# tingliu/glia

Hardware: AMD Instinct MI355X
Metric: region_merges_per_sec (higher is better)
Workload: dtype u32 labels / f32 image / f64 statistics and features

## Files before the change

### glia_amd/csrc/greedy.hip

```cpp
#include <atomic>
#include <cstring>
#include <vector>
#include <limits>
#include <rocprim/device/device_scan.hpp>
#include <rocprim/device/device_radix_sort.hpp>
#include <rocprim/device/device_segmented_radix_sort.hpp>

#include "greedy_batch.hpp"

namespace glia {

__global__ void pq_build_level_kernel(PqTree t, int l) {
  const int lane = threadIdx.x & 63;
  uint32_t j = (blockIdx.x * blockDim.x + threadIdx.x) >> 6;
  if (j < t.lv[l].size) (void)pq_recompute_node(t, l, j, lane, true);
}

int pq_setup(DeviceBuffers& buf, PqTree& t, hipStream_t stream) {
  t.nlevels = 0;
  uint32_t n = t.nleaves;
  while (true) {
    n = (n + kFan - 1) / kFan;
    if (t.nlevels >= kMaxLevels) { set_error("greedy: edge table too large"); return GLIA_HMT_ERR_ARG; }
    PqLevel& L = t.lv[t.nlevels++];
    L.size = n;
    int rc;
    if ((rc = buf.get(&L.sal, n, false, stream))) return rc;
    if ((rc = buf.get(&L.seq, n, false, stream))) return rc;
    if ((rc = buf.get(&L.arg, n, false, stream))) return rc;
    if ((rc = buf.get(&L.dirty, n, true, stream))) return rc;
    if (n <= kTopMax) break;
  }
  {
    int rc;
    if ((rc = buf.get(&t.glist[0], t.lv[0].size, false, stream))) return rc;
    if ((rc = buf.get(&t.glist[1], t.lv[0].size, false, stream))) return rc;
    if ((rc = buf.get(&t.gcount, 2, true, stream))) return rc;
  }
  for (int l = 0; l < t.nlevels; ++l) {
    unsigned long long threads = (unsigned long long)t.lv[l].size * 64ull;
    hipLaunchKernelGGL(pq_build_level_kernel, dim3((unsigned)((threads + 255) / 256)), dim3(256), 0, stream, t, l);
  }
  GLIA_HIP_TRY(hipGetLastError());
  return GLIA_HMT_OK;
}

namespace {

__global__ void win_range_kernel(const double* sal, uint32_t E0, unsigned long long* mm) {
  unsigned long long lo = ~0ull, hi = 0ull;
  for (uint32_t i = blockIdx.x * blockDim.x + threadIdx.x; i < E0; i += gridDim.x * blockDim.x) {
    const unsigned long long b = f64_ord(sal[i]);
    lo = b < lo ? b : lo; hi = b > hi ? b : hi;
  }
  atomicMin(&mm[0], lo); atomicMax(&mm[1], hi);
}
__global__ void win_params_kernel(const unsigned long long* mm, uint32_t B, double* range) {
  const double smin = f64_unord(mm[0]), smax = f64_unord(mm[1]);
  range[0] = smin;
  range[1] = smax > smin ? (double)B / (smax - smin) : 0.0;
}
__global__ void win_collect_kernel(const EdgeRec* er, uint32_t n_edges, const uint8_t* rdead, unsigned long long* kseq, uint32_t* vals, uint32_t* counter) {
  const uint32_t e = blockIdx.x * blockDim.x + threadIdx.x;
  if (e >= n_edges) return;
  const unsigned long long q = er[e].seq;
  if (q == 0) return;
  const uint2 uv = *reinterpret_cast<const uint2*>(&er[e].u);
  if (rdead[uv.x] | rdead[uv.y]) return;
  const uint32_t i = atomicAdd(counter, 1u);
  kseq[i] = q; vals[i] = e;
}
__global__ void win_salkey_kernel(const EdgeRec* er, const uint32_t* vals, uint32_t n, unsigned long long* ksal) {
  const uint32_t i = blockIdx.x * blockDim.x + threadIdx.x;
  if (i < n) ksal[i] = f64_ord(er[vals[i]].sal);
}
__global__ void win_baseline_fill_kernel(WinState st, uint32_t n, uint32_t* isort_w, unsigned long long* isort_seq) {
  const uint32_t i = blockIdx.x * blockDim.x + threadIdx.x;
  if (i >= n) return;
  const EdgeRec r = st.er[isort_w[i]];
  isort_seq[i] = r.seq;
  atomicAdd(&st.wcnt[win_cell(r.sal, st.wrange[0], st.wrange[1], st.wB)], 1u);
}
__global__ void win_segments_kernel(WinState st, const uint32_t* isort, uint32_t n, uint32_t* ige) {
  const uint32_t c = blockIdx.x * blockDim.x + threadIdx.x;
  if (c > st.wB) return;
  uint32_t lo = 0, hi = n;
  while (lo < hi) {
    const uint32_t mid = (lo + hi) >> 1;
    if (win_cell(st.er[isort[mid]].sal, st.wrange[0], st.wrange[1], st.wB) >= c) lo = mid + 1; else hi = mid;
  }
  ige[c] = c == 0 ? n : lo;
}
__global__ void adj_fill_fat(GreedyState g, WinState st, uint32_t E0, uint32_t* cursor) {
  const uint32_t e = blockIdx.x * blockDim.x + threadIdx.x;
  if (e >= E0) return;
  const uint32_t u = g.e_u[e], v = g.e_v[e];
  const uint32_t pu = atomicAdd(&cursor[u], 1u), pv = atomicAdd(&cursor[v], 1u);
  const uint32_t ou = g.adj_off[u], ov = g.adj_off[v], lu = g.adj_len[u], lv = g.adj_len[v];
  FatEntry a; a.eid = e; a.rs = v; a.n = (uint32_t)g.e_n[e]; a.pos = pv; a.off = ov; a.len = lv; a.mean = g.e_mean[e];
  FatEntry b = a; b.rs = u; b.pos = pu; b.off = ou; b.len = lu;
  st.fpool[ou + pu] = a; g.e_posu[e] = pu;
  st.fpool[ov + pv] = b; g.e_posv[e] = pv;
  EdgeRec r; r.u = u; r.v = v; r.posu = pu; r.posv = pv; r.mean = g.e_mean[e]; r.n = g.e_n[e]; r.next = kNone;
  r.hu = make_uint2(ou, lu); r.hv = make_uint2(ov, lv); r.sal = g.pq.leaf_sal[e]; r.seq = g.pq.leaf_seq[e];
  st.er[e] = r;
}
__global__ void fat_to_thin(const FatEntry* f, uint2* out, unsigned long long n) {
  const unsigned long long i = (unsigned long long)blockIdx.x * blockDim.x + threadIdx.x;
  if (i < n) { const FatEntry fe = f[i]; out[i] = make_uint2(fe.eid, fe.eid == kNone ? 0u : fe.rs); }
}
__global__ void edge_unpack(GreedyState g, const EdgeRec* er, const uint8_t* rdead, uint32_t n) {
  const uint32_t e = blockIdx.x * blockDim.x + threadIdx.x;
  if (e >= n) return;
  const EdgeRec r = er[e];
  g.e_u[e] = r.u; g.e_v[e] = r.v; g.e_posu[e] = r.posu; g.e_posv[e] = r.posv; g.e_mean[e] = r.mean; g.e_n[e] = r.n;
  g.pq.leaf_sal[e] = r.sal; g.pq.leaf_seq[e] = (rdead[r.u] | rdead[r.v]) ? 0ull : r.seq;
}

__global__ void edge_flags(const uint32_t* pa, const uint32_t* pb, long long P, uint32_t* flag, long long* partner) {
  long long i = (long long)blockIdx.x * blockDim.x + threadIdx.x;
  if (i >= P) return;
  uint32_t a = pa[i], b = pb[i];
  long long j = (a < b) ? find_pair(pa, pb, P, b, a) : -1;
  flag[i] = j >= 0 ? 1u : 0u;
  partner[i] = j;
}

__global__ void edge_fill(const uint32_t* pa, const uint32_t* pb, const uint32_t* prec, long long P,
                          const uint32_t* flag, const uint32_t* eidx, const long long* partner,
                          const uint32_t* rlabel, uint32_t R, GreedyState st, uint32_t* deg) {
  long long i = (long long)blockIdx.x * blockDim.x + threadIdx.x;
  if (i >= P || !flag[i]) return;
  const uint32_t e = eidx[i];
  const long long j = partner[i];
  const uint32_t u = find_label(rlabel, R, pa[i]), v = find_label(rlabel, R, pb[i]);
  const uint32_t* wi = &prec[(size_t)i * kPairWords];
  const uint32_t* wj = &prec[(size_t)j * kPairWords];
  double si, sj;
  memcpy(&si, &wi[P_SUM], 8);
  memcpy(&sj, &wj[P_SUM], 8);
  const int n = (int)(wi[P_CNT] + wj[P_CNT]);
  const double mean = sdivide(si + sj, (double)n, 0.0);
  st.e_u[e] = u; st.e_v[e] = v; st.e_mean[e] = mean; st.e_n[e] = n;
  st.pq.leaf_sal[e] = -mean; st.pq.leaf_seq[e] = (unsigned long long)e + 1ull;
  atomicAdd(&deg[u], 1u);
  atomicAdd(&deg[v], 1u);
}

__global__ void adj_fill(GreedyState st, uint32_t E0, uint32_t* cursor) {
  uint32_t e = blockIdx.x * blockDim.x + threadIdx.x;
  if (e >= E0) return;
  const uint32_t u = st.e_u[e], v = st.e_v[e];
  const uint32_t pu = atomicAdd(&cursor[u], 1u), pv = atomicAdd(&cursor[v], 1u);
  st.pool[st.adj_off[u] + pu] = make_uint2(e, v); st.e_posu[e] = pu;
  st.pool[st.adj_off[v] + pv] = make_uint2(e, u); st.e_posv[e] = pv;
}

__global__ void region_sizes(const uint32_t* rrec, uint32_t R, unsigned long long* rsz, double* rsum) {
  uint32_t r = blockIdx.x * blockDim.x + threadIdx.x;
  if (r >= R) return;
  const uint32_t* w = &rrec[(size_t)r * kRegionWords];
  rsz[r] = w[R_CNT];
  double d; memcpy(&d, &w[R_SUM], 8); rsum[r] = d;
}

__global__ void median_collect(VolumeRef vol, const uint32_t* pa, const uint32_t* pb, long long P, const uint32_t* flag,
                               const uint32_t* eidx, const unsigned long long* e_off, uint32_t* cursor, float* out) {
  const long long N = vol.nx * vol.ny * vol.nz;
  const long long p = (long long)blockIdx.x * blockDim.x + threadIdx.x;
  if (p >= N) return;
  const long long x = p % vol.nx, y = (p / vol.nx) % vol.ny, z = p / (vol.nx * vol.ny);
  const uint32_t t = vol.lab[p];
  if (t == kMaskedLabel) return;
  uint32_t nb = t;
  const long long sy = vol.nx, sz = vol.nx * vol.ny;
  const uint32_t* L = vol.lab_nb;
  do {
    uint32_t q;
    if (x > 0 && (q = L[p - 1]) != t && q != kMaskedLabel) { nb = q; break; }
    if (x + 1 < vol.nx && (q = L[p + 1]) != t && q != kMaskedLabel) { nb = q; break; }
    if (y > 0 && (q = L[p - sy]) != t && q != kMaskedLabel) { nb = q; break; }
    if (y + 1 < vol.ny && (q = L[p + sy]) != t && q != kMaskedLabel) { nb = q; break; }
    if (vol.dim == 3) {
      if (z > 0 && (q = L[p - sz]) != t && q != kMaskedLabel) { nb = q; break; }
      if (z + 1 < vol.nz && (q = L[p + sz]) != t && q != kMaskedLabel) { nb = q; break; }
    }
  } while (false);
  if (nb == t) return;
  const long long i = find_pair(pa, pb, P, t < nb ? t : nb, t < nb ? nb : t);
  if (i < 0 || !flag[i]) return;
  const uint32_t e = eidx[i];
  out[e_off[e] + atomicAdd(&cursor[e], 1u)] = vol.pb[p];
}

__global__ void median_from_runs(const unsigned long long* pv_off, const float* pv, unsigned long long nV, const uint32_t* pa, const uint32_t* pb, long long P,
                                 const uint32_t* flag, const uint32_t* eidx, const unsigned long long* e_off, float* out) {
  const unsigned long long v = (unsigned long long)blockIdx.x * blockDim.x + threadIdx.x;
  if (v >= nV) return;
  long long lo = 0, hi = P;
  while (lo < hi) { const long long mid = (lo + hi) >> 1; if (pv_off[mid + 1] <= v) lo = mid + 1; else hi = mid; }
  const long long i = lo;
  const uint32_t a = pa[i], b = pb[i];
  const long long owner = a < b ? i : find_pair(pa, pb, P, b, a);
  if (owner < 0 || !flag[owner]) return;
  const unsigned long long first = owner == i ? 0ull : pv_off[owner + 1] - pv_off[owner];
  out[e_off[eidx[owner]] + first + (v - pv_off[i])] = pv[v];
}

__global__ void median_init(GreedyState st, uint32_t E0) {
  const uint32_t e = blockIdx.x * blockDim.x + threadIdx.x;
  if (e >= E0) return;
  const uint32_t n = (uint32_t)st.e_n[e];
  const double med = (double)st.vals[st.e_off[e] + n / 2u];
  st.e_mean[e] = med;
  st.pq.leaf_sal[e] = st.size_weight ? -med * (double)min(st.rsz[st.e_u[e]], st.rsz[st.e_v[e]]) : -med;
  atomicAdd(&st.rbv[st.e_u[e]], (unsigned long long)n);
  atomicAdd(&st.rbv[st.e_v[e]], (unsigned long long)n);
}

__global__ void fill_leaves_dead(PqTree t, uint32_t from) {
  uint32_t i = from + blockIdx.x * blockDim.x + threadIdx.x;
  if (i < t.nleaves) { t.leaf_seq[i] = 0; t.leaf_sal[i] = -__builtin_inf(); }
}

}

struct WinBaseline {
  unsigned long long *kseq = nullptr, *kseq2 = nullptr, *ksal = nullptr, *ksal2 = nullptr, *iseq = nullptr;
  uint32_t *vals = nullptr, *vals2 = nullptr, *isort = nullptr, *ige = nullptr, *counter = nullptr;
  void* tmp = nullptr; size_t tmp_bytes = 0;
  uint32_t E0 = 0;
  double h_range[2] = {0.0, 0.0};
  long long prev_top_cell = -1;
  unsigned long long prev_ne = 0;
  double horizon_factor = 0.0;

  int init(DeviceBuffers& buf, WinState& ws, const double* leaf_sal, uint32_t n_initial, uint32_t B, uint32_t R, hipStream_t stream) {
    int rc;
    E0 = n_initial;
    unsigned long long* mm; double* range;
    if ((rc = buf.get(&ws.rdead, 2 * (size_t)R, true, stream))) return rc;
    if ((rc = buf.get(&ws.whead, B, false, stream))) return rc;
    if ((rc = buf.get(&ws.wcnt, B, true, stream))) return rc;
    if ((rc = buf.get(&isort, E0, false, stream))) return rc;
    if ((rc = buf.get(&iseq, E0, false, stream))) return rc;
    if ((rc = buf.get(&ige, (size_t)B + 1, false, stream))) return rc;
    if ((rc = buf.get(&mm, 2, false, stream))) return rc;
    if ((rc = buf.get(&range, 2, false, stream))) return rc;
    if ((rc = buf.get(&kseq, E0, false, stream))) return rc;
    if ((rc = buf.get(&kseq2, E0, false, stream))) return rc;
    if ((rc = buf.get(&ksal, E0, false, stream))) return rc;
    if ((rc = buf.get(&ksal2, E0, false, stream))) return rc;
    if ((rc = buf.get(&vals, E0, false, stream))) return rc;
    if ((rc = buf.get(&vals2, E0, false, stream))) return rc;
    if ((rc = buf.get(&counter, 1, true, stream))) return rc;
    GLIA_HIP_TRY(rocprim::radix_sort_pairs_desc(nullptr, tmp_bytes, kseq, kseq2, vals, vals2, (size_t)E0, 0, 64, stream));
    if ((rc = buf.get((char**)&tmp, tmp_bytes ? tmp_bytes : 16, false, stream))) return rc;
    ws.wrange = range; ws.isort = isort; ws.isort_seq = iseq; ws.ige = ige;
    const unsigned long long mm0[2] = {~0ull, 0ull};
    GLIA_HIP_TRY(hipMemcpyAsync(mm, mm0, sizeof(mm0), hipMemcpyHostToDevice, stream));
    hipLaunchKernelGGL(win_range_kernel, dim3(256), dim3(256), 0, stream, leaf_sal, E0, mm);
    hipLaunchKernelGGL(win_params_kernel, dim3(1), dim3(1), 0, stream, mm, B, range);
    GLIA_HIP_TRY(hipGetLastError());
    GLIA_HIP_TRY(hipMemcpyAsync(h_range, range, sizeof(h_range), hipMemcpyDeviceToHost, stream));
    GLIA_HIP_TRY(hipStreamSynchronize(stream));
    return GLIA_HMT_OK;
  }
  int rebaseline(WinState& ws, uint32_t n_edges, unsigned long long* ctrl, hipStream_t stream) {
    GLIA_HIP_TRY(hipMemsetAsync(counter, 0, sizeof(uint32_t), stream));
    hipLaunchKernelGGL(win_collect_kernel, dim3((n_edges + 255) / 256), dim3(256), 0, stream, ws.er, n_edges, ws.rdead, kseq, vals, counter);
    uint32_t n = 0;
    GLIA_HIP_TRY(hipMemcpyAsync(&n, counter, sizeof(uint32_t), hipMemcpyDeviceToHost, stream));
    GLIA_HIP_TRY(hipStreamSynchronize(stream));
    if (n > E0) { set_error("greedy: more live edges than initial edges (internal error)"); return GLIA_HMT_ERR_INTERNAL; }
    if (n) {
      size_t bytes = tmp_bytes;
      GLIA_HIP_TRY(rocprim::radix_sort_pairs_desc(tmp, bytes, kseq, kseq2, vals, vals2, (size_t)n, 0, 64, stream));
      hipLaunchKernelGGL(win_salkey_kernel, dim3((n + 255) / 256), dim3(256), 0, stream, ws.er, vals2, n, ksal);
      bytes = tmp_bytes;
      GLIA_HIP_TRY(rocprim::radix_sort_pairs_desc(tmp, bytes, ksal, ksal2, vals2, isort, (size_t)n, 0, 64, stream));
    }
    GLIA_HIP_TRY(hipMemsetAsync(ws.whead, 0xFF, sizeof(uint32_t) * ws.wB, stream));
    GLIA_HIP_TRY(hipMemsetAsync(ws.wcnt, 0, sizeof(uint32_t) * ws.wB, stream));
    if (n) hipLaunchKernelGGL(win_baseline_fill_kernel, dim3((n + 255) / 256), dim3(256), 0, stream, ws, n, isort, iseq);
    hipLaunchKernelGGL(win_segments_kernel, dim3((ws.wB + 1 + 255) / 256), dim3(256), 0, stream, ws, isort, n, ige);
    GLIA_HIP_TRY(hipGetLastError());
    ws.nsort = n;
    std::string renv;
    ws.rebase_after = option("GLIA_HMT_REBASE", &renv) ? strtoull(renv.c_str(), nullptr, 10) : std::max<unsigned long long>(800000ull, (unsigned long long)n / 2ull);
    ws.wch = 0;
    if (horizon_factor > 0.0 && n > 4096) {
      unsigned long long topkey = 0;
      GLIA_HIP_TRY(hipMemcpyAsync(&topkey, ksal2, sizeof(topkey), hipMemcpyDeviceToHost, stream));
      GLIA_HIP_TRY(hipStreamSynchronize(stream));
      const long long top_cell = (long long)win_cell(f64_unord(topkey), h_range[0], h_range[1], ws.wB);
      if (prev_top_cell >= 0 && n_edges > prev_ne) {
        const double d = (double)std::max<long long>(0, prev_top_cell - top_cell);
        const double delta = std::max(horizon_factor * d * (double)ws.rebase_after / (double)(n_edges - prev_ne), (double)ws.wB / 512.0);
        ws.wch = (double)top_cell > delta ? (uint32_t)((double)top_cell - delta) : 0u;
      }
      prev_top_cell = top_cell; prev_ne = n_edges;
    }
    ws.ne_base = n_edges;
    const double inf = std::numeric_limits<double>::infinity();
    ctrl[CTRL_CTHR] = (unsigned long long)(long long)(ws.wB - 1);
    memcpy(&ctrl[CTRL_TSAL], &inf, 8); ctrl[CTRL_TSEQ] = ~0ull; ctrl[CTRL_IPTR] = 0;
    return GLIA_HMT_OK;
  }
};

static int run_pb_loop(const RagArrays& rag, hipStream_t stream, const PbRequest& req, MergeResult* out) {
  const long long P = rag.P;
  const uint32_t R = (uint32_t)rag.R;
  if (R == 0 || P == 0) return GLIA_HMT_OK;
  const VolumeRef* median_of = req.median_of;
  CallEvents<3> ev;
  int rc;
  if ((rc = ev.create())) return rc;
  GLIA_HIP_TRY(hipEventRecord(ev.ev[0], stream));
  DeviceBuffers buf;
  uint32_t* flag; uint32_t* eidx; long long* partner;
  if ((rc = buf.get(&flag, P + 1, true, stream))) return rc;
  if ((rc = buf.get(&eidx, P + 1, false, stream))) return rc;
  if ((rc = buf.get(&partner, P, false, stream))) return rc;
  hipLaunchKernelGGL(edge_flags, dim3((unsigned)((P + 255) / 256)), dim3(256), 0, stream, rag.d_pa, rag.d_pb, P, flag, partner);
  if ((rc = rocprim_run(buf, stream, [&](void* t, size_t& b) {
        return rocprim::exclusive_scan(t, b, flag, eidx, 0u, (size_t)(P + 1), rocprim::plus<uint32_t>(), stream); }))) return rc;
  uint32_t E0 = 0;
  GLIA_HIP_TRY(hipMemcpyAsync(&E0, eidx + P, sizeof(uint32_t), hipMemcpyDeviceToHost, stream));
  GLIA_HIP_TRY(hipStreamSynchronize(stream));
  if (E0 == 0) return GLIA_HMT_OK;

  GreedyState st;
  memset(&st, 0, sizeof(st));
  st.R0 = R;
  const bool mincap = initial_capacities(E0, 18, 36, &st.Ecap, &st.pool_cap);
  if ((rc = buf.get(&st.adj_off, 2 * (size_t)R, true, stream))) return rc;
  if ((rc = buf.get(&st.adj_len, 2 * (size_t)R + 1, true, stream))) return rc;
  std::string o_window, o_batch, o_txt;
  const bool batch_off = option("GLIA_HMT_PB_BATCH", &o_batch) && o_batch[0] == '0';
  bool window = !median_of && !req.size_weight && !(option("GLIA_HMT_PB_WINDOW", &o_window) && o_window[0] == '0');
  WinState ws;
  memset(&ws, 0, sizeof(ws));
  GrowList edges, entries, values;
  if (window) {
    if ((rc = entries.add(buf, &ws.fpool, st.pool_cap, stream))) return rc;
    if ((rc = edges.add(buf, &ws.er, st.Ecap, stream))) return rc;
  }
  else if ((rc = entries.add(buf, &st.pool, st.pool_cap, stream))) return rc;
  if ((rc = edges.add(buf, &st.e_u, st.Ecap, stream)) || (rc = edges.add(buf, &st.e_v, st.Ecap, stream)) ||
      (rc = edges.add(buf, &st.e_posu, st.Ecap, stream)) || (rc = edges.add(buf, &st.e_posv, st.Ecap, stream)) ||
      (rc = edges.add(buf, &st.e_mean, st.Ecap, stream)) || (rc = edges.add(buf, &st.e_n, st.Ecap, stream, true)) ||
      (rc = edges.add(buf, &st.pq.leaf_sal, st.Ecap, stream)) || (rc = edges.add(buf, &st.pq.leaf_seq, st.Ecap, stream)))
    return rc;
  st.pq.nleaves = st.Ecap;
  if ((rc = buf.get(&st.rsz, 2 * (size_t)R, true, stream))) return rc;
  if ((rc = buf.get(&st.rsum, 2 * (size_t)R, true, stream))) return rc;
  st.cond_n = req.cond_n; st.cond_rpb = req.cond_rpb; st.size_weight = req.size_weight ? 1 : 0;
  st.cond_t0 = req.cond_n > 0 ? (unsigned long long)req.cond_sizes[0] : 0; st.cond_t1 = req.cond_n > 1 ? (unsigned long long)req.cond_sizes[1] : 0;
  hipLaunchKernelGGL(region_sizes, dim3((R + 255) / 256), dim3(256), 0, stream, rag.d_rrec, R, st.rsz, st.rsum);
  if ((rc = buf.get(&st.mark0, 2 * (size_t)R, true, stream))) return rc;
  if ((rc = buf.get(&st.mark1, 2 * (size_t)R, true, stream))) return rc;
  if ((rc = buf.get(&st.order, 3 * ((size_t)R + 16), false, stream))) return rc;
  if ((rc = buf.get(&st.sal_out, (size_t)R + 16, false, stream))) return rc;
  if ((rc = buf.get(&st.ctrl, 16, true, stream))) return rc;
  uint32_t* cursor;
  if ((rc = buf.get(&cursor, 2 * (size_t)R, true, stream))) return rc;

  hipLaunchKernelGGL(fill_leaves_dead, dim3((st.Ecap - E0 + 255) / 256), dim3(256), 0, stream, st.pq, E0);
  hipLaunchKernelGGL(edge_fill, dim3((unsigned)((P + 255) / 256)), dim3(256), 0, stream, rag.d_pa, rag.d_pb, rag.d_prec, P,
                     flag, eidx, partner, rag.d_rlabel, R, st, st.adj_len);
  if ((rc = rocprim_run(buf, stream, [&](void* t, size_t& b) {
        return rocprim::exclusive_scan(t, b, st.adj_len, st.adj_off, 0u, (size_t)R, rocprim::plus<uint32_t>(), stream); }))) return rc;
  if (window) hipLaunchKernelGGL(adj_fill_fat, dim3((E0 + 255) / 256), dim3(256), 0, stream, st, ws, E0, cursor);
  else hipLaunchKernelGGL(adj_fill, dim3((E0 + 255) / 256), dim3(256), 0, stream, st, E0, cursor);
  GLIA_HIP_TRY(hipGetLastError());
  unsigned long long n_values = 0;
  if (median_of) {
    if ((rc = edges.add(buf, &st.e_off, st.Ecap, stream))) return rc;
    if ((rc = buf.get(&st.rbv, 2 * (size_t)R, true, stream))) return rc;
    if ((rc = rocprim_run(buf, stream, [&](void* t, size_t& b) {
          return rocprim::exclusive_scan(t, b, st.e_n, st.e_off, 0ull, (size_t)E0 + 1, rocprim::plus<unsigned long long>(), stream); }))) return rc;
    GLIA_HIP_TRY(hipMemcpyAsync(&n_values, st.e_off + E0, sizeof(n_values), hipMemcpyDeviceToHost, stream));
    GLIA_HIP_TRY(hipStreamSynchronize(stream));
    if (n_values >= 0xFFFFFFFFull) { set_error("merge_order_pb: more than 2^32 boundary voxels (median linkage)"); return GLIA_HMT_ERR_ARG; }
    st.vals_cap = mincap ? std::max(n_values, 1ull) : n_values * 4ull + (1ull << 20);
    float* unsorted;
    if ((rc = values.add(buf, &st.vals, (size_t)st.vals_cap, stream))) return rc;
    if ((rc = buf.get(&unsorted, (size_t)n_values, false, stream))) return rc;
    uint32_t* vcursor;
    if ((rc = buf.get(&vcursor, (size_t)E0, true, stream))) return rc;
    if (median_of->lab) {
      const long long N = median_of->nx * median_of->ny * median_of->nz;
      hipLaunchKernelGGL(median_collect, dim3((unsigned)((N + 255) / 256)), dim3(256), 0, stream, *median_of, rag.d_pa, rag.d_pb, P,
                         flag, eidx, st.e_off, vcursor, unsorted);
    } else {
      if (!rag.d_pv_off) { set_error("merge_order_pb: median linkage needs the volume or the map's boundary values"); return GLIA_HMT_ERR_UNSUPPORTED; }
      if (rag.nV) hipLaunchKernelGGL(median_from_runs, dim3((unsigned)((rag.nV + 255) / 256)), dim3(256), 0, stream, rag.d_pv_off, rag.d_pv, rag.nV, rag.d_pa, rag.d_pb,
                                     (long long)P, flag, eidx, st.e_off, unsorted);
    }
    GLIA_HIP_TRY(hipGetLastError());
    if ((rc = rocprim_run(buf, stream, [&](void* t, size_t& b) {
          return rocprim::segmented_radix_sort_keys(t, b, unsorted, st.vals, (unsigned)n_values, (unsigned)E0, st.e_off, st.e_off + 1, 0, 32, stream); }))) return rc;
    hipLaunchKernelGGL(median_init, dim3((E0 + 255) / 256), dim3(256), 0, stream, st, E0);
    GLIA_HIP_TRY(hipGetLastError());
  }
  unsigned long long ctrl[CTRL_WORDS] = {};
  ctrl[CTRL_EDGES] = E0; ctrl[CTRL_ENTRIES] = 2ull * E0; ctrl[CTRL_STATUS] = ST_RUN; ctrl[CTRL_VALUES] = n_values;
  WinBaseline base;
  if (window) {
    uint32_t B = 256;
    while (B < E0 / 4 && B < (1u << 22)) B <<= 1;
    ws.wB = B; ws.R0 = R;
    ws.wcap = kWinCap; ws.wbudget = kWinBudget;
    ws.force_tree = 0;
    if (option("GLIA_HMT_FORCE_TREE", &o_txt)) ws.force_tree = strtoull(o_txt.c_str(), nullptr, 10);
    if (option("GLIA_HMT_WINCAP", &o_txt)) {
      const uint32_t c = (uint32_t)strtoul(o_txt.c_str(), nullptr, 10);
      if (c >= 16 && c <= kWinCap) { ws.wcap = c; ws.wbudget = c / 2; }
    }
    ws.order = st.order; ws.sal_out = st.sal_out; ws.ctrl = st.ctrl; ws.rsz = st.rsz; ws.rsum = st.rsum;
    ws.mark0 = st.mark0; ws.mark1 = st.mark1; ws.adj_off = st.adj_off; ws.adj_len = st.adj_len;
    ws.pool_cap = st.pool_cap; ws.Ecap = st.Ecap;
    ws.cond_n = st.cond_n; ws.cond_t0 = st.cond_t0; ws.cond_t1 = st.cond_t1; ws.cond_rpb = st.cond_rpb;
    if ((rc = base.init(buf, ws, st.pq.leaf_sal, E0, B, R, stream))) return rc;
    if (req.cond_n <= 0 && !batch_off) base.horizon_factor = option("GLIA_HMT_HORIZON", &o_txt) ? atof(o_txt.c_str()) : 0.5;
    if ((rc = base.rebaseline(ws, E0, ctrl, stream))) return rc;
  } else if ((rc = pq_setup(buf, st.pq, stream))) return rc;
  GLIA_HIP_TRY(hipMemcpyAsync(st.ctrl, ctrl, sizeof(ctrl), hipMemcpyHostToDevice, stream));
  GLIA_HIP_TRY(hipEventRecord(ev.ev[1], stream));


  st.max_iters = window ? 1ull << 22 : 1ull << 16;
  const bool trace = option("GLIA_HMT_TRACE");
  if (option("GLIA_HMT_MAXITERS", &o_txt)) st.max_iters = std::max(1ull, strtoull(o_txt.c_str(), nullptr, 10));
  const auto kernel = [&]() { return !window ? "tree" : req.cond_n > 0 ? "window" : "batch"; };
  const auto unhandled = [&]() {
    set_error(std::string("greedy: the ") + kernel() + " kernel stopped with status " + std::to_string(ctrl[CTRL_STATUS]) + ", which its driver does not handle (internal error)");
    return GLIA_HMT_ERR_INTERNAL;
  };
  while (true) {
    if (window) {
      ws.max_iters = st.max_iters;
      if (req.cond_n > 0) hipLaunchKernelGGL(greedy_window_kernel<true>, dim3(1), dim3(kGreedyThreads), 0, stream, ws);
      else if (batch_off) hipLaunchKernelGGL(greedy_window_kernel<false>, dim3(1), dim3(kGreedyThreads), 0, stream, ws);
      else hipLaunchKernelGGL(greedy_batch_kernel, dim3(1), dim3(kGreedyThreads), 0, stream, ws);
    } else if (median_of) hipLaunchKernelGGL(greedy_pb_kernel<true>, dim3(1), dim3(kGreedyThreads), 0, stream, st);
    else hipLaunchKernelGGL(greedy_pb_kernel<false>, dim3(1), dim3(kGreedyThreads), 0, stream, st);
    GLIA_HIP_TRY(hipGetLastError());
    GLIA_HIP_TRY(hipMemcpyAsync(ctrl, st.ctrl, sizeof(ctrl), hipMemcpyDeviceToHost, stream));
    GLIA_HIP_TRY(hipStreamSynchronize(stream));
    if (trace) fprintf(stderr, "[trace] merge loop launch ended: status %llu, merges %llu of %u regions, edges %llu, list entries %llu\n", ctrl[CTRL_STATUS], ctrl[CTRL_MERGES], R, ctrl[CTRL_EDGES], ctrl[CTRL_ENTRIES]);
    if (ctrl[CTRL_STATUS] == ST_DONE) break;
    switch (ctrl[CTRL_STATUS]) {
      case ST_RUN:
        if (!window) continue;
        break;
      case ST_REBASE:
        if (!window) return unhandled();
        break;
      case ST_BAD_SALIENCY: set_error("Error: invalid boundary saliency..."); return GLIA_HMT_ERR_SALIENCY;
      case ST_INTERNAL: {
        char msg[256];
        snprintf(msg, sizeof(msg), "greedy: window queue overflow or more merges than regions (internal error: merges %llu of %u regions, %llu edges of %u initial, "
                 "window %llu%s, %s kernel)", ctrl[CTRL_MERGES], R, ctrl[CTRL_EDGES], E0, ctrl[CTRL_WFILL], ctrl[CTRL_WERR] ? " overflowed" : "", kernel());
        set_error(msg);
        return GLIA_HMT_ERR_INTERNAL;
      }
      case ST_NEED_TREE:
        if (!window) return unhandled();
        entries.remove(&ws.fpool);
        edges.remove(&ws.er);
        if ((rc = entries.add(buf, &st.pool, st.pool_cap, stream))) return rc;
        hipLaunchKernelGGL(fat_to_thin, dim3((unsigned)((ctrl[CTRL_ENTRIES] + 255) / 256)), dim3(256), 0, stream, ws.fpool, st.pool, ctrl[CTRL_ENTRIES]);
        hipLaunchKernelGGL(edge_unpack, dim3((unsigned)((ctrl[CTRL_EDGES] + 255) / 256)), dim3(256), 0, stream, st, ws.er, ws.rdead, (uint32_t)ctrl[CTRL_EDGES]);
        GLIA_HIP_TRY(hipGetLastError());
        if ((rc = pq_setup(buf, st.pq, stream))) return rc;
        window = false;
        st.max_iters = 1ull << 16;
        break;
      case ST_NEED_POOL: {
        const unsigned long long ncap = st.pool_cap * 2;
        if ((rc = entries.grow(buf, (size_t)st.pool_cap, (size_t)ncap, stream))) return rc;
        st.pool_cap = ncap; ws.pool_cap = ncap;
        break;
      }
      case ST_NEED_VALUES: {
        if (!median_of) return unhandled();
        const unsigned long long ncap = st.vals_cap * 2;
        if ((rc = values.grow(buf, (size_t)ctrl[CTRL_VALUES], (size_t)ncap, stream))) return rc;
        st.vals_cap = ncap;
        break;
      }
      case ST_NEED_EDGES: {
        if (st.Ecap >= kMaxEdgeSlots) { set_error("greedy: more than 2^32 edge slots needed"); return GLIA_HMT_ERR_ARG; }
        const uint32_t ocap = st.Ecap, ncap = (uint32_t)std::min<unsigned long long>(kMaxEdgeSlots, (unsigned long long)ocap * 2ull);
        if ((rc = edges.grow(buf, ocap, ncap, stream))) return rc;
        st.Ecap = ncap; st.pq.nleaves = ncap; ws.Ecap = ncap;
        hipLaunchKernelGGL(fill_leaves_dead, dim3((ncap - ocap + 255) / 256), dim3(256), 0, stream, st.pq, ocap);
        if (!window && (rc = pq_setup(buf, st.pq, stream))) return rc;
        break;
      }
      default: return unhandled();
    }
    if (window) {
      if ((rc = base.rebaseline(ws, (uint32_t)ctrl[CTRL_EDGES], ctrl, stream))) return rc;
      GLIA_HIP_TRY(hipMemcpyAsync(st.ctrl + CTRL_CTHR, ctrl + CTRL_CTHR, 4 * sizeof(unsigned long long), hipMemcpyHostToDevice, stream));
    }
    unsigned long long zero = ST_RUN;
    GLIA_HIP_TRY(hipMemcpyAsync(st.ctrl + CTRL_STATUS, &zero, sizeof(zero), hipMemcpyHostToDevice, stream));
  }
  GLIA_HIP_TRY(hipEventRecord(ev.ev[2], stream));
  GLIA_HIP_TRY(hipEventSynchronize(ev.ev[2]));
  out->ms_table = ev.ms(0, 1); out->ms_loop = ev.ms(1, 2);
  out->n_scored = (int64_t)ctrl[CTRL_EDGES];
  return copy_merges(out, (int64_t)ctrl[CTRL_MERGES], st.order, st.sal_out);
}


static std::atomic<unsigned long long> g_internal_errors{0};
unsigned long long internal_errors() { return g_internal_errors.load(); }
void count_internal_error() { g_internal_errors.fetch_add(1); }
bool merge_order_is_consistent(const uint32_t* o, int64_t n, uint32_t R, int64_t* first_bad) {
  std::vector<uint8_t> gone(2 * (size_t)R + 1, 0);
  for (int64_t k = 0; k < n; ++k) {
    const uint32_t a = o[3 * k], b = o[3 * k + 1], c = o[3 * k + 2];
    if (k >= (int64_t)R || c != R + (uint32_t)k || a >= c || b >= c || a == b || gone[a] || gone[b]) { if (first_bad) *first_bad = k; return false; }
    gone[a] = gone[b] = 1;
  }
  return true;
}
int finish_merge_order(int rc, const uint32_t* o, int64_t n, uint32_t R, hipStream_t stream) {
  int64_t bad = -1;
  if (rc == GLIA_HMT_OK && !merge_order_is_consistent(o, n, R, &bad)) {
    set_error("greedy: merge " + std::to_string(bad) + " of " + std::to_string(n) + " joins a region that does not exist (any more) or creates the wrong one (internal error)");
    rc = GLIA_HMT_ERR_INTERNAL;
  }
  if (rc == GLIA_HMT_ERR_INTERNAL) { count_internal_error(); (void)hipStreamSynchronize(stream); }
  return rc;
}
int greedy_mean(const RagArrays& rag, hipStream_t stream, const PbRequest& req, MergeResult* out) {
  const int rc = run_pb_loop(rag, stream, req, out);
  return finish_merge_order(rc, out->order.data(), out->n, (uint32_t)rag.R, stream);
}

}
```

### glia_amd/csrc/greedy_batch.hpp

```cpp
#pragma once
#include "greedy_window.hpp"

namespace glia {
namespace {

constexpr uint32_t kBatchKill = 32;
constexpr int kMemP = 3;
constexpr uint32_t kMemMax = 192;
struct BatchShared {
  alignas(16) Key part1[kNW];
  alignas(16) Key part2[kNW];
  uint32_t nkill, kovf; alignas(16) uint32_t kill[kBatchKill];
  uint32_t byrank[kNW];
  uint32_t bitmap[kNW][64];
  uint32_t m_newcount[kNW], m_total[kNW], m_ok[kNW];
  double m_maxsal[kNW];
  uint32_t bad;
};

template <int CTRL, int ROW_MASK = 0xf>
__device__ __forceinline__ void top2_ord_step(unsigned long long& a1, unsigned long long& a2) {
  const unsigned long long b1 = dpp64<CTRL, ROW_MASK, ROW_MASK != 0xf>(a1), b2 = dpp64<CTRL, ROW_MASK, ROW_MASK != 0xf>(a2);
  const bool g = b1 > a1;
  const unsigned long long hi = g ? b1 : a1, lo = g ? a1 : b1, m2 = b2 > a2 ? b2 : a2;
  a1 = hi; a2 = lo > m2 ? lo : m2;
}
__device__ __forceinline__ void wave_top2_ord(unsigned long long& a1, unsigned long long& a2) {
  top2_ord_step<0xB1>(a1, a2);
  top2_ord_step<0x4E>(a1, a2);
  top2_ord_step<0x124>(a1, a2);
  top2_ord_step<0x128>(a1, a2);
  top2_ord_step<0x142, 0xa>(a1, a2);
  top2_ord_step<0x143, 0xc>(a1, a2);
  a1 = lane_u64(a1, 63); a2 = lane_u64(a2, 63);
}

#ifdef GLIA_HMT_PROFILE
__device__ unsigned long long g_scanprof[8];
__device__ unsigned long long g_scanfill[3][3];
#define SCAN_T(i) do { if (tid == 0) { const unsigned long long tn_ = __builtin_readcyclecounter(); g_scanprof[i] += tn_ - st_; st_ = tn_; } } while (0)
#else
#define SCAN_T(i) do {} while (0)
#endif
enum { kScanOther = 0, kScanNarrow = 1, kScanWide = 2 };
__device__ __forceinline__ void batch_scan(const WinState& st, WinShared& w, BatchShared& b, int tid, [[maybe_unused]] int from) {
#ifdef GLIA_HMT_PROFILE
  unsigned long long st_ = __builtin_readcyclecounter();
  if (tid == 0) g_scanprof[7] += 1;
#endif
  const uint32_t n = w.n < st.wcap ? w.n : st.wcap, nk = b.nkill < kBatchKill ? b.nkill : kBatchKill, kovf = b.kovf;
#ifdef GLIA_HMT_PROFILE
  if (tid == 0) g_scanfill[from][n <= 512u ? 0 : n <= 1024u ? 1 : 2] += 1;
#endif
  const uint32_t own = 64u * (uint32_t)(((tid >> 6) + (tid & 63)) & 7) + (uint32_t)(tid & 63);
  Key k1, k2;
  k1.sal = -__builtin_inf(); k1.seq = 0; k1.arg = 0; k2 = k1;
  auto pass = [&](auto nb_tag) {
    constexpr int NB = decltype(nb_tag)::value;
    unsigned long long q[NB]; uint32_t e[NB]; double sl[NB];
#pragma unroll
    for (int j = 0; j < NB; ++j) { const uint32_t i = own + (uint32_t)j * kGreedyThreads; q[j] = w.seq[i]; e[j] = w.e[i]; sl[j] = w.sal[i]; }
    const uint4 ka = *reinterpret_cast<const uint4*>(&b.kill[0]), kb = *reinterpret_cast<const uint4*>(&b.kill[4]);
    const uint32_t kl[8] = {ka.x, ka.y, ka.z, ka.w, kb.x, kb.y, kb.z, kb.w};
    SCAN_T(0);
    uint32_t deadm[NB];
#pragma unroll
    for (int j = 0; j < NB; ++j) {
      uint32_t d = 0;
#pragma unroll
      for (uint32_t t = 0; t < 8; ++t) d |= (uint32_t)(t < nk) & (uint32_t)(kl[t] == e[j]);
      deadm[j] = d;
    }
    if (nk > 8u) {
      for (uint32_t t = 8; t < nk; ++t) {
        const uint32_t kt = b.kill[t];
#pragma unroll
        for (int j = 0; j < NB; ++j) deadm[j] |= (uint32_t)(kt == e[j]);
      }
      if (kovf) {
        full_barrier();
#pragma unroll
        for (int j = 0; j < NB; ++j) {
          const uint32_t i = own + (uint32_t)j * kGreedyThreads;
          if (i < n && q[j] != 0) deadm[j] |= (uint32_t)(st.er[e[j]].seq == 0);
        }
      }
    }
#pragma unroll
    for (int j = 0; j < NB; ++j) {
      const uint32_t i = own + (uint32_t)j * kGreedyThreads;
      const bool was = (i < n) & (q[j] != 0);
      const bool live = was & (deadm[j] == 0u);
      if (was & !live) w.seq[i] = 0;
      Key c; c.sal = live ? sl[j] : -__builtin_inf(); c.seq = live ? q[j] : 0ull; c.arg = i;
      const bool b1 = better(c, k1), b2 = better(c, k2);
      k2.sal = b1 ? k1.sal : (b2 ? c.sal : k2.sal); k2.seq = b1 ? k1.seq : (b2 ? c.seq : k2.seq); k2.arg = b1 ? k1.arg : (b2 ? c.arg : k2.arg);
      k1.sal = b1 ? c.sal : k1.sal; k1.seq = b1 ? c.seq : k1.seq; k1.arg = b1 ? c.arg : k1.arg;
    }
  };
  static_assert(kWinPer == 3, "batch_scan: one pass instance per number of blocks");
  const uint32_t nu = (uint32_t)__builtin_amdgcn_readfirstlane((int)n);
  if (nu > 2u * kGreedyThreads) pass(std::integral_constant<int, 3>{});
  else if (nu > kGreedyThreads) pass(std::integral_constant<int, 2>{});
  else pass(std::integral_constant<int, 1>{});
  SCAN_T(1);
  const int lane = tid & 63;
  const unsigned long long o1 = f64_ord(k1.sal), o2 = f64_ord(k2.sal);
  unsigned long long M1 = o1, M2 = o2;
  wave_top2_ord(M1, M2);
  const unsigned long long t1 = __ballot(o1 == M1), t1l = __ballot((o1 == M1) & (k1.seq != 0ull));
  const int l1 = (int)__builtin_ctzll(t1);
  const bool win1 = lane == l1;
  Key kk; kk.sal = win1 ? k2.sal : k1.sal; kk.seq = win1 ? k2.seq : k1.seq; kk.arg = win1 ? k2.arg : k1.arg;
  const unsigned long long oc = win1 ? o2 : o1;
  const unsigned long long t2 = __ballot(oc == M2), t2l = __ballot((oc == M2) & (kk.seq != 0ull));
  Key m1, m2;
  if (__popcll(t1) == 1 || t1l == 0ull) {
    m1 = lane_key(k1, l1);
    int src = (int)__builtin_ctzll(t2);
    if (__popcll(t2) != 1 && t2l != 0ull) {
#ifdef GLIA_HMT_PROFILE
      if (tid == 0) g_scanprof[5] += 1;
#endif
      const unsigned long long ms = wave_max_u64(oc == M2 ? kk.seq : 0ull);
      src = (int)__builtin_ctzll(__ballot((oc == M2) & (kk.seq == ms)));
    }
    m2 = lane_key(kk, src);
    SCAN_T(2);
  } else {
#ifdef GLIA_HMT_PROFILE
    if (tid == 0) g_scanprof[6] += 1;
#endif
    unsigned long long S1 = o1 == M1 ? k1.seq : 0ull, S2 = o2 == M1 ? k2.seq : 0ull;
    wave_top2_ord(S1, S2);
    const int w1 = (int)__builtin_ctzll(__ballot((o1 == M1) & (k1.seq == S1)));
    const bool winr = lane == w1;
    Key kc; kc.sal = winr ? k2.sal : k1.sal; kc.seq = winr ? k2.seq : k1.seq; kc.arg = winr ? k2.arg : k1.arg;
    const unsigned long long occ = winr ? o2 : o1;
    m1 = lane_key(k1, w1);
    m2 = lane_key(kc, (int)__builtin_ctzll(__ballot((occ == M1) & (kc.seq == S2))));
    SCAN_T(3);
  }
  if ((tid & 63) == 0) { b.part1[tid >> 6] = m1; b.part2[tid >> 6] = m2; }
  full_barrier();
  SCAN_T(4);
  if (tid == 0) { b.nkill = 0; b.kovf = 0; }
}

#ifdef GLIA_HMT_PROFILE
__device__ unsigned long long g_wideprof[8];
#define WIDE_T(i) do { if (tid == 0) { const unsigned long long tn_ = __builtin_readcyclecounter(); g_wideprof[i] += tn_ - wt_; wt_ = tn_; } } while (0)
#else
#define WIDE_T(i) do {} while (0)
#endif
__device__ __forceinline__ uint32_t batch_contract_wide(const WinState& st, WinShared& w, WinWork& s, BatchShared& b, int tid, uint32_t slot, double rootsal,
                                                      unsigned long long k, unsigned long long ne, unsigned long long pool_used, double smin, double scale, uint32_t* newcount_out) {
  const uint32_t e = w.e[slot], r0 = w.u[slot], r1 = w.v[slot];
  const uint2 h0r = w.hu[slot], h1r = w.hv[slot];
  const uint32_t wn_now = w.n;
  const uint32_t off0 = h0r.x, len0 = h0r.y, off1 = h1r.x, len1 = h1r.y;
  const uint32_t total = len0 + len1;
  const uint32_t r2 = st.R0 + (uint32_t)k;
  const uint32_t r2off = (uint32_t)pool_used;
#ifdef GLIA_HMT_PROFILE
  unsigned long long wt_ = __builtin_readcyclecounter();
#endif
  lds_barrier();
  WIDE_T(0);
  if (tid == 0) {
    w.seq[slot] = 0;
    st.order[3 * k + 0] = r0; st.order[3 * k + 1] = r1; st.order[3 * k + 2] = r2;
    st.sal_out[k] = rootsal;
    st.er[e].seq = 0;
    st.rdead[r0] = 1; st.rdead[r1] = 1;
  }
  const bool small = total <= kMarkMax;
  win_stage_lists(st, s, tid, e, off0, len0, off1, len1, small);
  if (small) lds_barrier(); else full_barrier();
  WIDE_T(1);
  if (wn_now + total > st.wcap && wn_now > st.wcap / 2u) win_compact(w, tid, st.wcap);
  WIDE_T(2);
  const WinTau tau = {w.cthr, w.tsal, w.tseq, smin, scale};
  const uint32_t nwork = small ? s.nitems : total;
  const uint32_t lenR2 = small ? nwork : 0u;
  bool bad = false;
  uint32_t pend_e = kNone, pend_old = kNone;
  auto rounds = [&](auto small_tag) {
    constexpr bool SMALL = decltype(small_tag)::value;
    for (uint32_t base = 0; base < nwork; base += kGreedyThreads) {
      const uint32_t i = base + tid;
      if (i >= nwork) break;
      FatEntry f0, f1;
      bool h0, h1;
      uint32_t rs;
      if (!win_match<SMALL>(st, s, i, e, off0, len0, off1, &rs, &h0, &h1, &f0, &f1)) continue;
      const uint32_t idx = atomicAdd(&s.newcount, 1u);
      const uint32_t newE = (uint32_t)ne + idx;
      double first;
      int second;
      if (mean_link(h0, f0.mean, (int)f0.n, h1, f1.mean, (int)f1.n, &first, &second)) bad = true;
      const uint32_t offRs = f0.off, posRs = f0.pos, lenRs = f0.len;
      if (h0 && h1) st.fpool[offRs + f1.pos].eid = kNone;
      const unsigned long long seq = update_seq(k, rs, r0, h0);
      const double sal = -first;
      store_new_edge(st, newE, rs, r2, posRs, idx, first, second, sal, seq, offRs, lenRs, r2off, lenR2);
      win_queue_edge<true>(st, w, tau, newE, sal, seq, rs, r2, make_uint2(offRs, lenRs), make_uint2(r2off, lenR2), pend_e, pend_old);
      if (h0) win_retire_edge<true, false, kBatchKill>(st, tau, f0.eid, -f0.mean, &b.nkill, b.kill, &b.kovf);
      if (h1) win_retire_edge<true, false, kBatchKill>(st, tau, f1.eid, -f1.mean, &b.nkill, b.kill, &b.kovf);
    }
  };
  if (small) rounds(std::true_type{}); else rounds(std::false_type{});
  if (bad) b.bad = 1;
  WIDE_T(3);
  if (small) lds_barrier(); else full_barrier();
  WIDE_T(4);
  const uint32_t newcount = s.newcount;
  if (!small) win_complete_r2(st, tid, (uint32_t)ne, r2off, newcount);
  if (!small) for (uint32_t i = tid; i < (w.n < st.wcap ? w.n : st.wcap); i += kGreedyThreads) if (w.v[i] == r2) w.hv[i].y = newcount;
  if (pend_e != kNone) st.er[pend_e].next = pend_old;
  if (tid == 0) { st.adj_off[r2] = r2off; st.adj_len[r2] = newcount; }
  lds_barrier();
  WIDE_T(5);
  if (tid == 0) { s.nitems = 0; s.newcount = 0; }
  *newcount_out = newcount;
  return total;
}

__global__ __launch_bounds__(kGreedyThreads) void greedy_batch_kernel(WinState st) {
  __shared__ WinShared w;
  __shared__ WinWork s;
  __shared__ BatchShared b;
  const int tid = threadIdx.x, lane = tid & 63, wave = tid >> 6;
  unsigned long long k = st.ctrl[CTRL_MERGES], ne = st.ctrl[CTRL_EDGES], pool_used = st.ctrl[CTRL_ENTRIES];
  uint32_t status = ST_RUN;
  win_enter(st, w, s, tid);
  if (tid == 0) { b.nkill = 0; b.kovf = 0; b.bad = 0; }
  b.bitmap[wave][lane] = 0;
  if (tid < kNW) { Key z; z.sal = -__builtin_inf(); z.seq = 0; z.arg = 0; b.part1[tid] = z; b.part2[tid] = z; }
  full_barrier();
  const double smin = st.wrange[0], scale = st.wrange[1];
  uint32_t pend_e = kNone, pend_old = kNone;
  constexpr uint32_t kTab = kMarkSlots / kNW;
  uint32_t* const tk = &s.mk[wave * kTab]; uint32_t* const t0 = &s.mv0[wave * kTab]; uint32_t* const t1 = &s.mv1[wave * kTab];
  static_assert(sizeof(s.stage) >= (size_t)kNW * kTab * 20, "per-wave staging");
  uint32_t* const sg_eid = reinterpret_cast<uint32_t*>(&s.stage[0]) + wave * kTab;
  uint32_t* const sg_n = reinterpret_cast<uint32_t*>(&s.stage[0]) + (kNW + wave) * kTab;
  uint32_t* const sg_pos = reinterpret_cast<uint32_t*>(&s.stage[0]) + (2 * kNW + wave) * kTab;
  double* const sg_mean = reinterpret_cast<double*>(reinterpret_cast<uint32_t*>(&s.stage[0]) + 3 * kNW * kTab) + wave * kTab;
#ifdef GLIA_HMT_PROFILE
  unsigned long long bph[8] = {0, 0, 0, 0, 0, 0, 0, 0}, blast = __builtin_readcyclecounter(), brounds = 0, bmembers = 0, bvalid = 0, bwide = 0, bcut_sal = 0, bcut_dep = 0;
  unsigned long long bw_n[4] = {0, 0, 0, 0}, bw_cyc[4] = {0, 0, 0, 0}, bw_ent[4] = {0, 0, 0, 0}, bw_new[4] = {0, 0, 0, 0};
  unsigned long long bsel[2] = {0, 0}, bsel_n[2] = {0, 0};
#define BPH0(wide) do { if (tid == 0) { unsigned long long tn = __builtin_readcyclecounter(); bph[0] += tn - blast; bsel[wide] += tn - blast; bsel_n[wide] += 1; blast = tn; } } while (0)
#define BPH(i) do { if (tid == 0) { unsigned long long tn = __builtin_readcyclecounter(); bph[i] += tn - blast; blast = tn; } } while (0)
#else
#define BPH(i) do {} while (0)
#define BPH0(wide) do {} while (0)
#endif

  for (unsigned long long it = 0; it < st.max_iters; ++it) {
    if (ne - st.ne_base > st.rebase_after) { status = ST_REBASE; break; }
    const int gi = lane >> 3, gj = lane & 7;
    const Key A = b.part1[gi], B = b.part1[gj], C = b.part2[gi];
    const unsigned long long beats = __ballot(better(A, B)), under = __ballot(better(C, B));
    const unsigned long long col = 0x0101010101010101ull << gj;
    const uint32_t rank = (uint32_t)__popcll(beats & col);
    const bool cand_ok = B.seq != 0 && (under & col) == 0;
    if (gi == 0 && cand_ok) b.byrank[rank] = (uint32_t)gj;
    const unsigned long long okmask = __ballot(gi == 0 && cand_ok);
    const uint32_t M = (uint32_t)__popcll(okmask);
    if (M == 0) {
      BPH(5);
      if (pend_e != kNone) { st.er[pend_e].next = pend_old; pend_e = kNone; }
      if (st.force_tree && k >= st.force_tree) { status = ST_NEED_TREE; break; }
      const int r = win_reload(st, w, tid, reinterpret_cast<double*>(&s.stage[0]), reinterpret_cast<unsigned long long*>(&s.stage[0]) + kSelMax);
      BPH(6);
      if (r == 1) { status = ST_DONE; break; }
      if (r == 2) { status = ST_NEED_TREE; break; }
      if (r == 3) { status = ST_REBASE; break; }
      batch_scan(st, w, b, tid, kScanOther);
      continue;
    }
    const unsigned long long minemask = __ballot(gi == 0 && cand_ok && rank == (uint32_t)wave);
    const bool member = minemask != 0;
    const int cj = member ? (int)__builtin_ctzll(minemask) : 0;
    const Key me = b.part1[cj];
    const uint32_t slot = me.arg;
    const uint32_t e = w.e[slot], r0 = w.u[slot], r1 = w.v[slot];
    const uint2 h0r = w.hu[slot], h1r = w.hv[slot];
    const uint32_t off0 = h0r.x, len0 = h0r.y, off1 = h1r.x, len1 = h1r.y;
    const uint32_t total = len0 + len1;
    if (k >= (unsigned long long)st.R0) { status = ST_INTERNAL; break; }
    const unsigned long long firstmask = __ballot(gi == 0 && cand_ok && rank == 0u);
    const Key top = b.part1[__builtin_ctzll(firstmask)];
    const uint2 th0 = w.hu[top.arg], th1 = w.hv[top.arg];
    const uint32_t top_total = th0.y + th1.y;
    BPH0(top_total > kMemMax ? 1 : 0);
    if (top_total > kMemMax) {
      if (ne + top_total > st.Ecap) { status = ST_NEED_EDGES; break; }
      if (pool_used + top_total > st.pool_cap) { status = ST_NEED_POOL; break; }
      uint32_t newcount = 0;
#ifdef GLIA_HMT_PROFILE
      const unsigned long long tw0 = __builtin_readcyclecounter();
#endif
      const uint32_t tt = batch_contract_wide(st, w, s, b, tid, top.arg, top.sal, k, ne, pool_used, smin, scale, &newcount);
      if (b.bad) { status = ST_BAD_SALIENCY; break; }
      k += 1; ne += newcount; pool_used += tt;
#ifdef GLIA_HMT_PROFILE
      bwide += 1;
      { const int cls = tt <= 512u ? 0 : tt <= kMarkMax ? 1 : tt <= 8192u ? 2 : 3; bw_n[cls] += 1; bw_cyc[cls] += __builtin_readcyclecounter() - tw0; bw_ent[cls] += tt; bw_new[cls] += newcount; }
#endif
      batch_scan(st, w, b, tid, kScanWide);
      if (w.spill_ord) { if (pend_e != kNone) { st.er[pend_e].next = pend_old; pend_e = kNone; } win_evict(st, w, tid); batch_scan(st, w, b, tid, kScanOther); }
      BPH(4);
      continue;
    }
    const bool narrow = member && total <= kMemMax;
    b.bitmap[wave][lane] = 0;
    FatEntry fe[kMemP];
    bool act[kMemP], side1[kMemP];
    uint32_t h[kMemP];
#pragma unroll
    for (int p = 0; p < kMemP; ++p) {
      const uint32_t i = (uint32_t)lane + 64u * (uint32_t)p;
      const bool inlist = narrow && i < total;
      side1[p] = i >= len0;
      fe[p].eid = kNone; fe[p].rs = 0; fe[p].n = 0; fe[p].pos = 0; fe[p].off = 0; fe[p].len = 0; fe[p].mean = 0.0;
      if (inlist) fe[p] = st.fpool[side1[p] ? off1 + (i - len0) : off0 + i];
      act[p] = inlist;
    }
    if (pend_e != kNone) { st.er[pend_e].next = pend_old; pend_e = kNone; }
#pragma unroll
    for (int p = 0; p < kMemP; ++p) {
      act[p] = act[p] && fe[p].eid != e && fe[p].eid != kNone;
      h[p] = (fe[p].rs * 2654435761u) >> 24;
      if (act[p]) {
        while (true) {
          const uint32_t old = atomicCAS(&tk[h[p]], 0u, fe[p].rs + 1u);
          if (old == 0u || old == fe[p].rs + 1u) break;
          h[p] = (h[p] + 1u) & (kTab - 1u);
        }
        if (side1[p]) {
          t1[h[p]] = 1u;
          sg_eid[h[p]] = fe[p].eid; sg_n[h[p]] = fe[p].n; sg_pos[h[p]] = fe[p].pos; sg_mean[h[p]] = fe[p].mean;
        } else t0[h[p]] = 1u;
        atomicOr(&b.bitmap[wave][(fe[p].rs >> 5) & 63u], 1u << (fe[p].rs & 31u));
      }
    }
    if (narrow && lane == 0) { atomicOr(&b.bitmap[wave][(r0 >> 5) & 63u], 1u << (r0 & 31u)); atomicOr(&b.bitmap[wave][(r1 >> 5) & 63u], 1u << (r1 & 31u)); }
    asm volatile("s_waitcnt lgkmcnt(0)" ::: "memory");
    bool owner[kMemP], both[kMemP];
    uint32_t p_eid[kMemP], p_n[kMemP], p_pos[kMemP];
    double p_mean[kMemP];
#pragma unroll
    for (int p = 0; p < kMemP; ++p) {
      const uint32_t m0 = act[p] ? t0[h[p]] : 0u, m1 = act[p] ? t1[h[p]] : 0u;
      owner[p] = act[p] && (!side1[p] || m0 == 0u);
      both[p] = owner[p] && !side1[p] && m1 != 0u;
      p_eid[p] = sg_eid[h[p]]; p_n[p] = sg_n[h[p]]; p_pos[p] = sg_pos[h[p]]; p_mean[p] = sg_mean[h[p]];
    }
#pragma unroll
    for (int p = 0; p < kMemP; ++p) if (act[p]) { tk[h[p]] = 0u; t0[h[p]] = 0u; t1[h[p]] = 0u; }
    double first[kMemP]; int second[kMemP]; uint32_t idx[kMemP];
    bool bad = false;
    uint32_t newcount = 0;
    double mx = -__builtin_inf();
#pragma unroll
    for (int p = 0; p < kMemP; ++p) {
      const bool h0 = owner[p] && !side1[p], h1 = owner[p] && (side1[p] || both[p]);
      bad = mean_link(h0, fe[p].mean, (int)fe[p].n, h1, both[p] ? p_mean[p] : fe[p].mean, both[p] ? (int)p_n[p] : (int)fe[p].n, &first[p], &second[p]) || bad;
      const double f = first[p];
      const unsigned long long ownmask = __ballot(owner[p]);
      idx[p] = newcount + (uint32_t)__popcll(ownmask & ((1ull << lane) - 1ull));
      newcount += (uint32_t)__popcll(ownmask);
      mx = (owner[p] && -f > mx) ? -f : mx;
    }
#pragma unroll
    for (int d = 32; d >= 1; d >>= 1) { const double o = __shfl_xor(mx, d); mx = o > mx ? o : mx; }
    if (lane == 0) { b.m_newcount[wave] = narrow ? newcount : 0u; b.m_total[wave] = narrow ? total : 0xFFFFFFFFu; b.m_maxsal[wave] = mx; }
    if (bad) b.bad = 1;
    const uint32_t wn_round = w.n;
    lds_barrier();
    BPH(1);
    if (b.bad) { status = ST_BAD_SALIENCY; break; }
    uint32_t V, ne_off, pool_off, my_ne, my_pool;
    {
      const uint32_t j = (uint32_t)lane & 7u;
      const Key kj = b.part1[b.byrank[j]];
      const uint32_t u = w.u[kj.arg], v = w.v[kj.arg];
      const uint32_t tj = b.m_total[j], nj = b.m_newcount[j];
      double pm = -__builtin_inf();
      uint32_t hit = 0, pre_n = 0, pre_t = 0;
#pragma unroll
      for (uint32_t i = 0; i < (uint32_t)kNW; ++i) {
        const double ms = b.m_maxsal[i];
        const uint32_t bu = b.bitmap[i][(u >> 5) & 63u], bv = b.bitmap[i][(v >> 5) & 63u];
        const uint32_t ti = b.m_total[i], ni = b.m_newcount[i];
        if (i < j) { pm = ms > pm ? ms : pm; hit |= ((bu >> (u & 31u)) | (bv >> (v & 31u))) & 1u; pre_n += ni; pre_t += ti; }
      }
      const bool okj = j < M && tj != 0xFFFFFFFFu && (j == 0u || (kj.sal > pm && hit == 0u));
      const uint32_t okbits = (uint32_t)(__ballot(lane < kNW && okj) & 0xFFull);
      V = (uint32_t)__builtin_ctz(~okbits);
#ifdef GLIA_HMT_PROFILE
      if (V < M) { const uint32_t cutsal = (uint32_t)(__ballot(lane < kNW && j == V && !(kj.sal > pm)) & 0xFFull); if (cutsal) bcut_sal += 1; else bcut_dep += 1; }
#endif
      my_ne = (uint32_t)__builtin_amdgcn_readlane((int)pre_n, wave); my_pool = (uint32_t)__builtin_amdgcn_readlane((int)pre_t, wave);
      const uint32_t last = V - 1u;
      ne_off = (uint32_t)__shfl((int)(pre_n + nj), (int)last); pool_off = (uint32_t)__shfl((int)(pre_t + tj), (int)last);
    }
    const uint32_t sum_tot = pool_off;
    if (ne + sum_tot > st.Ecap) { status = ST_NEED_EDGES; break; }
    if (pool_used + sum_tot > st.pool_cap) { status = ST_NEED_POOL; break; }
    bool popped = false;
    if (wn_round + ne_off > st.wcap && wn_round > st.wcap / 2u) {
      if ((uint32_t)wave < V && lane == 0) w.seq[slot] = 0;
      popped = true;
      lds_barrier();
      win_compact(w, tid, st.wcap);
    }
    const WinTau tau = {w.cthr, w.tsal, w.tseq, smin, scale};
    BPH(2);
    if ((uint32_t)wave < V) {
      const unsigned long long kk = k + (unsigned long long)wave;
      const uint32_t r2 = st.R0 + (uint32_t)kk;
      const uint32_t r2off = (uint32_t)pool_used + my_pool;
      if (lane == 0) {
        if (!popped) w.seq[slot] = 0;
        st.order[3 * kk + 0] = r0; st.order[3 * kk + 1] = r1; st.order[3 * kk + 2] = r2;
        st.sal_out[kk] = me.sal;
        st.er[e].seq = 0;
        st.rdead[r0] = 1; st.rdead[r1] = 1;
        st.adj_off[r2] = r2off; st.adj_len[r2] = newcount;
      }
#pragma unroll
      for (int p = 0; p < kMemP; ++p) {
        if (!owner[p]) continue;
        const bool h0 = !side1[p];
        const uint32_t rs = fe[p].rs;
        const uint32_t newE = (uint32_t)ne + my_ne + idx[p];
        const uint32_t offRs = fe[p].off, posRs = fe[p].pos, lenRs = fe[p].len;
        if (both[p]) st.fpool[offRs + p_pos[p]].eid = kNone;
        const unsigned long long seq = update_seq(kk, rs, r0, h0);
        const double sal = -first[p];
        store_new_edge(st, newE, rs, r2, posRs, idx[p], first[p], second[p], sal, seq, offRs, lenRs, r2off, newcount);
        win_queue_edge<true>(st, w, tau, newE, sal, seq, rs, r2, make_uint2(offRs, lenRs), make_uint2(r2off, newcount), pend_e, pend_old);
        win_retire_edge<true, false, kBatchKill>(st, tau, fe[p].eid, -fe[p].mean, &b.nkill, b.kill, &b.kovf);
        if (both[p]) win_retire_edge<true, false, kBatchKill>(st, tau, p_eid[p], -p_mean[p], &b.nkill, b.kill, &b.kovf);
      }
    }
    lds_barrier();
    BPH(3);
#ifdef GLIA_HMT_PROFILE
    brounds += 1; bmembers += M; bvalid += V;
#endif
    k += V; ne += ne_off; pool_used += pool_off;
    batch_scan(st, w, b, tid, kScanNarrow);
    if (w.spill_ord) { if (pend_e != kNone) { st.er[pend_e].next = pend_old; pend_e = kNone; } win_evict(st, w, tid); batch_scan(st, w, b, tid, kScanOther); }
    BPH(4);
  }
#ifdef GLIA_HMT_PROFILE
  if (tid == 0) printf("[batch profile] merges %llu: select %llu  compute %llu  validate %llu  commit %llu  scan %llu  loop-top %llu  reload %llu (cycles); rounds %llu candidates %llu committed %llu (cut by saliency %llu, by adjacency %llu) wide %llu\n",
                       k, bph[0], bph[1], bph[2], bph[3], bph[4], bph[5], bph[6], brounds, bmembers, bvalid, bcut_sal, bcut_dep, bwide);
  if (tid == 0) printf("[batch profile] scan phases (cumulative cycles, wave 0): loads %llu  compare %llu  top2 %llu  top2 with a tied best %llu  barrier %llu  calls %llu  tied second %llu  tied best %llu\n",
                       g_scanprof[0], g_scanprof[1], g_scanprof[2], g_scanprof[3], g_scanprof[4], g_scanprof[7], g_scanprof[5], g_scanprof[6]);
  if (tid == 0) printf("[batch profile] scan fill (cumulative; n <= 512, <= 1024, more): after reload/evict %llu %llu %llu  after narrow round %llu %llu %llu  after wide %llu %llu %llu\n",
                       g_scanfill[0][0], g_scanfill[0][1], g_scanfill[0][2], g_scanfill[1][0], g_scanfill[1][1], g_scanfill[1][2], g_scanfill[2][0], g_scanfill[2][1], g_scanfill[2][2]);
  if (tid == 0) printf("[batch profile] loop top (this launch): narrow rounds %llu cycles %llu  wide pops %llu cycles %llu\n", bsel_n[0], bsel[0], bsel_n[1], bsel[1]);
  if (tid == 0) printf("[batch profile] wide phases (cumulative cycles): entry-barrier %llu  lists+table %llu  compact %llu  main loop (wave 0) %llu  loop barrier %llu  tail %llu\n",
                       g_wideprof[0], g_wideprof[1], g_wideprof[2], g_wideprof[3], g_wideprof[4], g_wideprof[5]);
  if (tid == 0) printf("[batch profile] wide by entries (<=512, <=1408, <=8192, more): n %llu %llu %llu %llu  cycles %llu %llu %llu %llu  entries %llu %llu %llu %llu  new edges %llu %llu %llu %llu\n",
                       bw_n[0], bw_n[1], bw_n[2], bw_n[3], bw_cyc[0], bw_cyc[1], bw_cyc[2], bw_cyc[3], bw_ent[0], bw_ent[1], bw_ent[2], bw_ent[3], bw_new[0], bw_new[1], bw_new[2], bw_new[3]);
#endif
  if (pend_e != kNone) st.er[pend_e].next = pend_old;
  full_barrier();
  win_leave(st, w, tid, k, ne, pool_used, status);
}

}
}
```

### glia_amd/csrc/greedy_window.hpp

```cpp
#pragma once
#include "greedy_tree.hpp"

namespace glia {

struct __attribute__((aligned(16))) FatEntry {
  uint32_t eid;
  uint32_t rs;
  uint32_t n;
  uint32_t pos;
  uint32_t off;
  uint32_t len;
  double mean;
};

namespace {

struct __attribute__((aligned(16))) EdgeRec {
  uint32_t u, v, posu, posv;
  double mean; int n; uint32_t next;
  uint2 hu, hv;
  double sal; unsigned long long seq;
};
static_assert(sizeof(EdgeRec) == 64, "EdgeRec layout");
struct WinState {
  EdgeRec* er; FatEntry* fpool;
  uint32_t* whead;
  uint32_t* wcnt;
  const uint32_t* isort; const unsigned long long* isort_seq;
  const uint32_t* ige;
  const double* wrange;
  uint32_t* order; double* sal_out; unsigned long long* ctrl;
  unsigned long long* rsz; double* rsum; uint32_t *mark0, *mark1, *adj_off, *adj_len;
  unsigned long long pool_cap, max_iters, cond_t0, cond_t1;
  double cond_rpb;
  uint32_t R0, Ecap, wB, nsort;
  unsigned long long ne_base, rebase_after;
  uint32_t wcap, wbudget;
  int cond_n;
  uint32_t wch;
  uint8_t* rdead;
  unsigned long long force_tree;
};
constexpr uint32_t kWinCap = 1536;
constexpr uint32_t kWinBudget = 768;
constexpr uint32_t kWinMinLoad = 192;
constexpr uint32_t kWinMinPartial = 96;
constexpr uint32_t kKillMax = 8;
constexpr int kNW = kGreedyThreads / 64;
constexpr int kWinPer = (int)(kWinCap / kGreedyThreads);
static_assert(kWinPer * kGreedyThreads == (int)kWinCap, "window capacity");
struct WinShared {
  double sal[kWinCap];
  unsigned long long seq[kWinCap];
  uint32_t e[kWinCap], u[kWinCap], v[kWinCap];
  uint2 hu[kWinCap], hv[kWinCap];
  int cthr; uint32_t iptr;
  double tsal; unsigned long long tseq;
  alignas(16) uint32_t n;
  uint32_t nk, kovf, pad0;
  alignas(16) uint32_t kill[kKillMax];
  alignas(16) Key part[kNW];
  uint32_t touched[2][64];
  uint32_t wsum[kNW];
  uint32_t bcast, maxcell, err, need_tree;
  double psal; unsigned long long pseq;
  unsigned long long spill_ord;
};
struct WinWork {
  uint32_t mk[kMarkSlots], mv0[kMarkSlots], mv1[kMarkSlots];
  uint32_t items[kMarkMax], newidx[kMarkMax], nitems, newcount, bad;
  FatEntry stage[kMarkMax];
};

__host__ __device__ __forceinline__ uint32_t win_cell(double sal, double smin, double scale, uint32_t B) {
  double t = (sal - smin) * scale;
  t = t > 0.0 ? t : 0.0;
  return t >= (double)(B - 1u) ? B - 1u : (uint32_t)t;
}
__device__ __forceinline__ bool win_above(int cthr, double tsal, unsigned long long tseq, int cell, double sal, unsigned long long seq) {
  return cell > cthr || (cell == cthr && (sal > tsal || (sal == tsal && seq > tseq)));
}

__device__ __forceinline__ uint32_t block_scan_incl(uint32_t v, uint32_t* wsum, int tid, uint32_t* total) {
  const int lane = tid & 63, wave = tid >> 6;
  uint32_t x = v;
#pragma unroll
  for (int d = 1; d < 64; d <<= 1) { const uint32_t y = (uint32_t)__shfl_up((int)x, d); if (lane >= d) x += y; }
  full_barrier();
  if (lane == 63) wsum[wave] = x;
  full_barrier();
  uint32_t base = 0, tot = 0;
#pragma unroll
  for (int i = 0; i < kNW; ++i) { const uint32_t s = wsum[i]; if (i < wave) base += s; tot += s; }
  *total = tot;
  return base + x;
}

__device__ __forceinline__ void win_put(WinShared& w, uint32_t slot, double sal, unsigned long long seq, uint32_t e, uint32_t u, uint32_t v, uint2 hu, uint2 hv) {
  w.sal[slot] = sal; w.seq[slot] = seq; w.e[slot] = e; w.u[slot] = u; w.v[slot] = v; w.hu[slot] = hu; w.hv[slot] = hv;
}
__device__ __forceinline__ void win_take(const WinState& st, WinShared& w, uint32_t e, const EdgeRec& r) {
  if (r.seq != 0) {
    const uint32_t slot = atomicAdd(&w.n, 1u);
    if (slot < st.wcap) win_put(w, slot, r.sal, r.seq, e, r.u, r.v, r.hu, r.hv); else w.err = 1;
  }
}

__device__ __forceinline__ void win_scan(const WinState& st, WinShared& w, int tid, uint32_t r2, uint32_t r2len) {
  const uint4 hd = *reinterpret_cast<const uint4*>(&w.n);
  const uint4 k0 = *reinterpret_cast<const uint4*>(&w.kill[0]), k1 = *reinterpret_cast<const uint4*>(&w.kill[4]);
  unsigned long long q[kWinPer]; uint32_t e[kWinPer], v[kWinPer]; double sl[kWinPer];
#pragma unroll
  for (int j = 0; j < kWinPer; ++j) { const uint32_t i = (uint32_t)tid + (uint32_t)j * kGreedyThreads; q[j] = w.seq[i]; e[j] = w.e[i]; v[j] = w.v[i]; sl[j] = w.sal[i]; }
  const uint32_t n = hd.x, nk = hd.y < kKillMax ? hd.y : kKillMax;
  const uint32_t kl[kKillMax] = {k0.x, k0.y, k0.z, k0.w, k1.x, k1.y, k1.z, k1.w};
  Key k;
  k.sal = -__builtin_inf(); k.seq = 0; k.arg = 0;
#pragma unroll
  for (int j = 0; j < kWinPer; ++j) {
    const uint32_t i = (uint32_t)tid + (uint32_t)j * kGreedyThreads;
    bool live = i < n && q[j] != 0;
    bool dead = false;
    if (nk) {
#pragma unroll
      for (uint32_t t = 0; t < kKillMax; ++t) dead = dead || (t < nk && kl[t] == e[j]);
    }
    if (live && hd.z) dead = dead || st.er[e[j]].seq == 0;
    if (live && dead) { w.seq[i] = 0; live = false; }
    if (live && v[j] == r2) w.hv[i].y = r2len;
    Key c; c.sal = live ? sl[j] : -__builtin_inf(); c.seq = live ? q[j] : 0ull; c.arg = i;
    if (better(c, k)) k = c;
  }
  k = wave_max(k);
  if ((tid & 63) == 0) w.part[tid >> 6] = k;
  lds_barrier();
  if (tid == 0) { w.nk = 0; w.kovf = 0; }
}
__device__ __forceinline__ Key win_root(const WinShared& w, int lane) {
  static_assert(kNW == 8, "win_root");
  Key k = w.part[lane & (kNW - 1)];
  key_max_step<0xB1>(k); key_max_step<0x4E>(k);
  const Key a = lane_key(k, 0), b = lane_key(k, 4);
  return better(b, a) ? b : a;
}

__device__ __forceinline__ uint32_t win_compact(WinShared& w, int tid, uint32_t cap = kWinCap) {
  double sal[kWinPer]; unsigned long long seq[kWinPer]; uint32_t e[kWinPer], u[kWinPer], v[kWinPer]; uint2 hu[kWinPer], hv[kWinPer];
  uint32_t live = 0;
  const uint32_t n = w.n < cap ? w.n : cap;
#pragma unroll
  for (int j = 0; j < kWinPer; ++j) {
    const uint32_t i = (uint32_t)tid * kWinPer + j;
    seq[j] = i < n ? w.seq[i] : 0ull;
    sal[j] = w.sal[i]; e[j] = w.e[i]; u[j] = w.u[i]; v[j] = w.v[i]; hu[j] = w.hu[i]; hv[j] = w.hv[i];
    live += seq[j] != 0;
  }
  uint32_t total;
  uint32_t o = block_scan_incl(live, w.wsum, tid, &total) - live;
#pragma unroll
  for (int j = 0; j < kWinPer; ++j) if (seq[j] != 0) { win_put(w, o, sal[j], seq[j], e[j], u[j], v[j], hu[j], hv[j]); ++o; }
  if (tid == 0) w.n = total;
  full_barrier();
  return total;
}

__device__ __forceinline__ void win_push_global(const WinState& st, uint32_t e, uint32_t cell) {
  const uint32_t old = atomicExch(&st.whead[cell], e);
  st.er[e].next = old;
  atomicAdd(&st.wcnt[cell], 1u);
}

__device__ __forceinline__ void win_flush(const WinState& st, WinShared& w, int tid) {
  const double smin = st.wrange[0], scale = st.wrange[1];
  if (tid == 0) w.maxcell = 0;
  full_barrier();
  const uint32_t n = w.n < st.wcap ? w.n : st.wcap;
  uint32_t mc = 0;
  for (uint32_t i = tid; i < n; i += kGreedyThreads) {
    if (w.seq[i] == 0) continue;
    const uint32_t c = win_cell(w.sal[i], smin, scale, st.wB);
    win_push_global(st, w.e[i], c);
    mc = mc > c + 1u ? mc : c + 1u;
  }
  if (mc) atomicMax(&w.maxcell, mc);
  full_barrier();
  if (tid == 0) {
    if (w.maxcell && (int)w.maxcell - 1 >= w.cthr) { w.cthr = (int)w.maxcell - 1; w.tsal = __builtin_inf(); w.tseq = ~0ull; }
    w.n = 0;
  }
  full_barrier();
}

__device__ __forceinline__ void win_evict(const WinState& st, WinShared& w, int tid) {
  const double smin = st.wrange[0], scale = st.wrange[1];
  const double lim = f64_unord(w.spill_ord);
  const uint32_t n = w.n < st.wcap ? w.n : st.wcap;
  full_barrier();
  for (uint32_t i = tid; i < n; i += kGreedyThreads) {
    if (w.seq[i] == 0 || w.sal[i] > lim) continue;
    win_push_global(st, w.e[i], win_cell(w.sal[i], smin, scale, st.wB));
    w.seq[i] = 0;
  }
  full_barrier();
  if (tid == 0) { w.n = n; w.cthr = (int)win_cell(lim, smin, scale, st.wB); w.tsal = lim; w.tseq = ~0ull; w.spill_ord = 0; }
  full_barrier();
}

__device__ __forceinline__ void win_take_initial(const WinState& st, WinShared& w, uint32_t a, uint32_t b, int tid) {
  for (uint32_t i = a + (uint32_t)tid; i < b; i += kGreedyThreads) { const uint32_t e = st.isort[i]; const EdgeRec r = st.er[e]; win_take(st, w, e, r); }
}

constexpr uint32_t kSelMax = 384;
__device__ __forceinline__ int win_reload(const WinState& st, WinShared& w, int tid, double* sel_sal, unsigned long long* sel_seq) {
  full_barrier();
  if (tid == 0) { w.n = 0; w.need_tree = 0; }
  full_barrier();
  uint32_t c_hi = (uint32_t)(w.cthr + 1) < st.wB ? (uint32_t)(w.cthr + 1) : st.wB, loaded = 0, iptr = w.iptr;
  int result = 1;
  const uint32_t c_floor = st.wch < st.wB ? st.wch : 0u;
  while (c_hi > c_floor) {
    const bool valid = (uint32_t)tid < c_hi - c_floor;
    const uint32_t c = valid ? c_hi - 1u - (uint32_t)tid : 0u;
    const uint32_t cn = valid ? ld_relaxed(&st.wcnt[c]) : 0u;
    uint32_t total;
    const uint32_t incl = block_scan_incl(cn, w.wsum, tid, &total);
    const bool ok = valid && incl <= st.wbudget - loaded;
    const uint32_t m = (uint32_t)__syncthreads_count(ok ? 1 : 0);
    const uint32_t nvalid = c_hi - c_floor < (uint32_t)kGreedyThreads ? c_hi - c_floor : (uint32_t)kGreedyThreads;
    if (m != 0) {
      const uint32_t c_lo = c_hi - m;
      if ((uint32_t)tid == m - 1u) w.bcast = incl;
      const uint32_t i_to = st.ige[c_lo];
      win_take_initial(st, w, iptr, i_to, tid);
      iptr = i_to > iptr ? i_to : iptr;
      if ((uint32_t)tid < m) {
        uint32_t e = ld_relaxed(&st.whead[c]);
        if (e != kNone) {
          st_agent(&st.whead[c], kNone);
          if (cn != 0) while (e != kNone) { const EdgeRec r = st.er[e]; win_take(st, w, e, r); e = r.next; }
        }
        if (cn != 0) st_agent(&st.wcnt[c], 0u);
      }
      full_barrier();
      loaded += w.bcast;
      c_hi = c_lo;
      if (loaded) result = 0;
    }
    if (m < nvalid) {
      const uint32_t room = st.wbudget - loaded;
      const uint32_t cs = c_hi - 1u;
      if (room >= (kWinMinPartial < st.wbudget / 8u ? kWinMinPartial : st.wbudget / 8u) || loaded == 0) {
        const uint32_t K = (room / 2u < kSelMax ? room / 2u : kSelMax) > 1u ? (room / 2u < kSelMax ? room / 2u : kSelMax) : 2u, RA = room > K ? room - K : 1u;
        const uint32_t seg_end = st.ige[cs];
        const uint32_t before = w.n;
        if (tid == 0) {
          uint32_t hn = 0, nlive = 0;
          for (uint32_t e = ld_relaxed(&st.whead[cs]); e != kNone;) {
            const EdgeRec r = st.er[e];
            if (r.seq != 0) {
              ++nlive;
              if (hn < K) {
                uint32_t i = hn++;
                while (i > 0) {
                  const uint32_t p = (i - 1u) >> 1;
                  if (!(sel_sal[p] > r.sal || (sel_sal[p] == r.sal && sel_seq[p] > r.seq))) break;
                  sel_sal[i] = sel_sal[p]; sel_seq[i] = sel_seq[p]; i = p;
                }
                sel_sal[i] = r.sal; sel_seq[i] = r.seq;
              } else if (r.sal > sel_sal[0] || (r.sal == sel_sal[0] && r.seq > sel_seq[0])) {
                uint32_t i = 0;
                while (true) {
                  uint32_t c = 2u * i + 1u;
                  if (c >= hn) break;
                  if (c + 1u < hn && (sel_sal[c + 1u] < sel_sal[c] || (sel_sal[c + 1u] == sel_sal[c] && sel_seq[c + 1u] < sel_seq[c]))) ++c;
                  if (!(sel_sal[c] < r.sal || (sel_sal[c] == r.sal && sel_seq[c] < r.seq))) break;
                  sel_sal[i] = sel_sal[c]; sel_seq[i] = sel_seq[c]; i = c;
                }
                sel_sal[i] = r.sal; sel_seq[i] = r.seq;
              }
            }
            e = r.next;
          }
          w.psal = nlive > K ? sel_sal[0] : -__builtin_inf(); w.pseq = nlive > K ? sel_seq[0] : 0ull;
        }
        full_barrier();
        double tsal = w.psal; unsigned long long tseq = w.pseq;
        const uint32_t iA = seg_end > iptr ? (seg_end - iptr < RA ? seg_end : iptr + RA) : iptr;
        if (iA < seg_end) {
          const uint32_t et = st.isort[iA]; const double as = st.er[et].sal; const unsigned long long aq = st.isort_seq[iA];
          if (as > tsal || (as == tsal && aq > tseq)) { tsal = as; tseq = aq; }
        }
        if (tid == 0) w.bcast = 0;
        full_barrier();
        uint32_t mine = 0;
        for (uint32_t i = iptr + (uint32_t)tid; i < iA; i += kGreedyThreads) {
          const uint32_t e = st.isort[i]; const EdgeRec r = st.er[e];
          const unsigned long long q = st.isort_seq[i];
          if (r.sal > tsal || (r.sal == tsal && q > tseq)) { ++mine; win_take(st, w, e, r); }
        }
        if (mine) atomicAdd(&w.bcast, mine);
        full_barrier();
        iptr += w.bcast;
        if (tid == 0) {
          uint32_t keep_head = kNone, keep_tail = kNone;
          for (uint32_t e = ld_relaxed(&st.whead[cs]); e != kNone;) {
            const EdgeRec r = st.er[e];
            if (r.seq != 0) {
              if (r.sal > tsal || (r.sal == tsal && r.seq > tseq)) win_take(st, w, e, r);
              else { if (keep_head == kNone) keep_head = e; else st.er[keep_tail].next = e; keep_tail = e; }
            }
            e = r.next;
          }
          if (keep_tail != kNone) st.er[keep_tail].next = kNone;
          st_agent(&st.whead[cs], keep_head);
        }
        full_barrier();
        const uint32_t moved = w.n - before;
        if (moved == 0u && w.bcast == 0u) {
          full_barrier();
          if (tid == 0) st_agent(&st.wcnt[cs], 0u);
          c_hi = cs;
          continue;
        }
        if (tid == 0) { if (moved) atomicSub(&st.wcnt[cs], moved); w.cthr = (int)cs; w.tsal = tsal; w.tseq = tseq; w.iptr = iptr; }
        if (moved || w.bcast) result = 0;
        full_barrier();
        return result;
      }
      break;
    }
    if (loaded >= (kWinMinLoad < st.wbudget / 4u ? kWinMinLoad : st.wbudget / 4u)) break;
  }
  full_barrier();
  if (tid == 0 && result != 2) { w.cthr = (int)c_hi - 1; w.tsal = __builtin_inf(); w.tseq = ~0ull; w.iptr = iptr; }
  full_barrier();
  if (result == 1 && c_floor != 0u) result = 3;
  return result;
}

struct WinTau { int cthr; double tsal; unsigned long long tseq; double smin, scale; };

__device__ __forceinline__ void win_stage_lists(const WinState& st, WinWork& s, int tid, uint32_t e, uint32_t off0, uint32_t len0, uint32_t off1, uint32_t len1, bool small) {
  const uint32_t total = len0 + len1;
  for (uint32_t i = tid; i < total; i += kGreedyThreads) {
    const bool side1 = i >= len0;
    const FatEntry fe = st.fpool[side1 ? off1 + (i - len0) : off0 + i];
    if (fe.eid == e || fe.eid == kNone) continue;
    if (small) {
      s.stage[i] = fe;
      uint32_t h = (fe.rs * 2654435761u) >> 21;
      while (true) {
        const uint32_t old = atomicCAS(&s.mk[h], 0u, fe.rs + 1u);
        if (old == 0u) { s.items[atomicAdd(&s.nitems, 1u)] = h; break; }
        if (old == fe.rs + 1u) break;
        h = (h + 1u) & (kMarkSlots - 1u);
      }
      (side1 ? s.mv1 : s.mv0)[h] = i + 1u;
    } else (side1 ? st.mark1 : st.mark0)[fe.rs] = i + 1u;
  }
}
template <bool SMALL>
__device__ __forceinline__ bool win_match(const WinState& st, WinWork& s, uint32_t i, uint32_t e, uint32_t off0, uint32_t len0, uint32_t off1,
                                          uint32_t* rs, bool* h0, bool* h1, FatEntry* f0, FatEntry* f1) {
  if constexpr (SMALL) {
    const uint32_t h = s.items[i];
    *rs = s.mk[h] - 1u;
    const uint32_t m0 = s.mv0[h], m1 = s.mv1[h];
    s.mk[h] = 0u; s.mv0[h] = 0u; s.mv1[h] = 0u;
    *h0 = m0 != 0; *h1 = m1 != 0;
    *f0 = s.stage[*h0 ? m0 - 1u : m1 - 1u]; *f1 = s.stage[*h1 ? m1 - 1u : m0 - 1u];
  } else {
    const bool side1 = i >= len0;
    const FatEntry fe = st.fpool[side1 ? off1 + (i - len0) : off0 + i];
    if (fe.eid == e || fe.eid == kNone) return false;
    *rs = fe.rs;
    if (!side1) {
      const uint32_t m = st.mark1[fe.rs];
      *h0 = true; *h1 = m != 0; *f0 = fe;
      *f1 = *h1 ? st.fpool[off1 + (m - 1u - len0)] : fe;
    } else {
      if (st.mark0[fe.rs] != 0u) return false;
      *h0 = false; *h1 = true; *f0 = fe; *f1 = fe;
    }
  }
  return true;
}
__device__ __forceinline__ void store_new_edge(const WinState& st, uint32_t newE, uint32_t rs, uint32_t r2, uint32_t posRs, uint32_t idx, double first, int second,
                                               double sal, unsigned long long seq, uint32_t offRs, uint32_t lenRs, uint32_t r2off, uint32_t lenR2) {
  uint4* pq4 = reinterpret_cast<uint4*>(&st.er[newE]);
  pq4[0] = make_uint4(rs, r2, posRs, idx);
  const unsigned long long mb = (unsigned long long)__double_as_longlong(first);
  pq4[1] = make_uint4((uint32_t)mb, (uint32_t)(mb >> 32), (uint32_t)second, kNone);
  pq4[2] = make_uint4(offRs, lenRs, r2off, lenR2);
  const unsigned long long sbits = (unsigned long long)__double_as_longlong(sal);
  pq4[3] = make_uint4((uint32_t)sbits, (uint32_t)(sbits >> 32), (uint32_t)seq, (uint32_t)(seq >> 32));
  FatEntry a; a.eid = newE; a.rs = r2; a.n = (uint32_t)second; a.pos = idx; a.off = r2off; a.len = lenR2; a.mean = first;
  st.fpool[offRs + posRs] = a;
  FatEntry b; b.eid = newE; b.rs = rs; b.n = (uint32_t)second; b.pos = posRs; b.off = offRs; b.len = lenRs; b.mean = first;
  st.fpool[r2off + idx] = b;
}
template <bool BATCH>
__device__ __forceinline__ void win_queue_edge(const WinState& st, WinShared& w, const WinTau& tau, uint32_t newE, double sal, unsigned long long seq, uint32_t rs, uint32_t r2,
                                               uint2 hrs, uint2 hr2, uint32_t& pend_e, uint32_t& pend_old) {
  const uint32_t cell = win_cell(sal, tau.smin, tau.scale, st.wB);
  const bool above = win_above(tau.cthr, tau.tsal, tau.tseq, (int)cell, sal, seq);
  uint32_t sl = kWinCap;
  if (above) {
    sl = atomicAdd(&w.n, 1u);
    if (!BATCH || sl < st.wcap) win_put(w, sl, sal, seq, newE, rs, r2, hrs, hr2);
    else atomicMax(&w.spill_ord, f64_ord(sal));
  }
  if (BATCH ? (sl >= st.wcap && (above || cell >= st.wch)) : !above) {
    if (pend_e != kNone) st.er[pend_e].next = pend_old;
    pend_e = newE; pend_old = atomicExch(&st.whead[cell], newE);
    atomicAdd(&st.wcnt[cell], 1u);
  }
}
template <bool BATCH, bool COND, uint32_t KMAX>
__device__ __forceinline__ void win_retire_edge(const WinState& st, const WinTau& tau, uint32_t de, double dsal, uint32_t* nkill, uint32_t* kill, uint32_t* kovf) {
  const uint32_t dc = win_cell(dsal, tau.smin, tau.scale, st.wB);
  const bool tie = (int)dc == tau.cthr && dsal == tau.tsal;
  unsigned long long dq = BATCH ? 0ull : 1ull;
  if (BATCH && dc < st.wch) return;
  if (!BATCH && (COND || tie)) dq = st.er[de].seq;
  st.er[de].seq = 0;
  if (!BATCH && dq == 0) return;
  if ((BATCH && tie) || win_above(tau.cthr, tau.tsal, tau.tseq, (int)dc, dsal, dq)) {
    const uint32_t j = atomicAdd(nkill, 1u); if (j < KMAX) kill[j] = de; else *kovf = 1;
  } else atomicSub(&st.wcnt[dc], 1u);
}
__device__ __forceinline__ void win_complete_r2(const WinState& st, int tid, uint32_t ne, uint32_t r2off, uint32_t newcount) {
  for (uint32_t j = tid; j < newcount; j += kGreedyThreads) {
    const FatEntry fb = st.fpool[r2off + j];
    st.fpool[fb.off + fb.pos].len = newcount;
    st.er[ne + j].hv.y = newcount;
    st.mark0[fb.rs] = 0; st.mark1[fb.rs] = 0;
  }
}
__device__ __forceinline__ void win_enter(const WinState& st, WinShared& w, WinWork& s, int tid) {
  if (tid == 0) {
    w.n = 0; w.nk = 0; w.kovf = 0; w.err = 0; w.spill_ord = 0; s.nitems = 0; s.newcount = 0; s.bad = 0;
    w.cthr = (int)(long long)st.ctrl[CTRL_CTHR]; w.tsal = __longlong_as_double((long long)st.ctrl[CTRL_TSAL]); w.tseq = st.ctrl[CTRL_TSEQ]; w.iptr = (uint32_t)st.ctrl[CTRL_IPTR];
  }
  for (uint32_t i = tid; i < kMarkSlots; i += kGreedyThreads) { s.mk[i] = 0; s.mv0[i] = 0; s.mv1[i] = 0; }
  for (uint32_t i = tid; i < kWinCap; i += kGreedyThreads) { w.seq[i] = 0; w.e[i] = 0; w.v[i] = 0; w.sal[i] = 0.0; }
}
__device__ __forceinline__ void win_leave(const WinState& st, WinShared& w, int tid, unsigned long long k, unsigned long long ne, unsigned long long pool_used, uint32_t status) {
  win_flush(st, w, tid);
  if (tid == 0) {
    st.ctrl[CTRL_MERGES] = k; st.ctrl[CTRL_EDGES] = ne; st.ctrl[CTRL_ENTRIES] = pool_used;
    st.ctrl[CTRL_STATUS] = w.err ? (unsigned long long)ST_INTERNAL : status; st.ctrl[CTRL_WERR] = w.err; st.ctrl[CTRL_WFILL] = w.n;
    st.ctrl[CTRL_CTHR] = (unsigned long long)(long long)w.cthr; st.ctrl[CTRL_TSAL] = (unsigned long long)__double_as_longlong(w.tsal); st.ctrl[CTRL_TSEQ] = w.tseq; st.ctrl[CTRL_IPTR] = w.iptr;
  }
}

template <bool COND>
__global__ __launch_bounds__(kGreedyThreads) void greedy_window_kernel(WinState st) {
  __shared__ WinShared w;
  __shared__ WinWork s;
  const int tid = threadIdx.x, lane = tid & 63;
  unsigned long long k = st.ctrl[CTRL_MERGES], ne = st.ctrl[CTRL_EDGES], pool_used = st.ctrl[CTRL_ENTRIES];
  uint32_t status = ST_RUN;
  win_enter(st, w, s, tid);
  if (tid < 128) w.touched[tid >> 6][tid & 63] = 0;
  if (tid < kNW) { w.part[tid].sal = -__builtin_inf(); w.part[tid].seq = 0; w.part[tid].arg = 0; }
  full_barrier();
  const double smin = st.wrange[0], scale = st.wrange[1];
  uint32_t r2prev = kNone;
#ifdef GLIA_HMT_PROFILE
  unsigned long long wph[8] = {0, 0, 0, 0, 0, 0, 0, 0}, wlast = __builtin_readcyclecounter(), wtiter = wlast;
  unsigned long long wtb[5] = {0, 0, 0, 0, 0}, wnb[5] = {0, 0, 0, 0, 0}, wdb[5] = {0, 0, 0, 0, 0}, wreloads = 0, wcompacts = 0, wloaded = 0, winwin = 0, wdeps = 0;
#define WPH(i) do { if (tid == 0) { unsigned long long tn = __builtin_readcyclecounter(); wph[i] += tn - wlast; wlast = tn; } } while (0)
#else
#define WPH(i) do {} while (0)
#endif

  for (unsigned long long it = 0; it < st.max_iters; ++it) {
    const Key root = win_root(w, lane);
    if (root.seq == 0) {
      WPH(5);
      if (st.force_tree && k >= st.force_tree) { status = ST_NEED_TREE; break; }
      const int r = win_reload(st, w, tid, reinterpret_cast<double*>(&s.stage[0]), reinterpret_cast<unsigned long long*>(&s.stage[0]) + kSelMax);
#ifdef GLIA_HMT_PROFILE
      wreloads += 1; wloaded += w.n;
#endif
      WPH(6);
      if (r == 1) { status = ST_DONE; break; }
      if (r == 2) { status = ST_NEED_TREE; break; }
      if (r == 3) { status = ST_REBASE; break; }
      win_scan(st, w, tid, kNone, 0);
      r2prev = kNone;
      continue;
    }
    const uint32_t slot = root.arg;
    const uint32_t e = w.e[slot], r0 = w.u[slot], r1 = w.v[slot];
    const uint2 h0r = w.hu[slot], h1r = w.hv[slot];
    const uint32_t wn_now = w.n;
    const int cthr = w.cthr; const double tsal = w.tsal; const unsigned long long tseq = w.tseq;
    const uint32_t off0 = h0r.x, len0 = h0r.y, off1 = h1r.x, len1 = h1r.y;
    const uint32_t total = len0 + len1;
    if (k >= (unsigned long long)st.R0) { status = ST_INTERNAL; break; }
    const uint32_t r2 = st.R0 + (uint32_t)k;
    const uint32_t r2off = (uint32_t)pool_used;
    const int par = (int)(k & 1ull);
    const uint32_t tb0 = w.touched[par ^ 1][(r0 >> 5) & 63u], tb1 = w.touched[par ^ 1][(r1 >> 5) & 63u];
    const bool dep = r2prev != kNone && (r1 == r2prev || r0 == r2prev || ((tb0 >> (r0 & 31u)) & 1u) || ((tb1 >> (r1 & 31u)) & 1u));
    if (dep) {
      full_barrier();
#ifdef GLIA_HMT_PROFILE
      wdeps += 1;
#endif
    }
    WPH(0);
    if (COND) {
      unsigned long long sz0 = st.rsz[r0], sz1 = st.rsz[r1]; double su0 = st.rsum[r0], su1 = st.rsum[r1];
      const unsigned long long z2 = sz0 + sz1; const double w2 = su0 + su1;
      if (sz0 > sz1) { const unsigned long long t = sz0; sz0 = sz1; sz1 = t; const double d = su0; su0 = su1; su1 = d; }
      bool ok = sz0 < st.cond_t0;
      if (!ok && st.cond_n > 1) {
        if (sz0 < st.cond_t1 && sdivide(su0, (double)sz0, 0.0) > st.cond_rpb) ok = true;
        if (!ok && sz1 < st.cond_t1 && sdivide(su1, (double)sz1, 0.0) > st.cond_rpb) ok = true;
      }
      if (!ok) {
        full_barrier();
        if (tid == 0) { w.seq[slot] = 0; st.er[e].seq = 0; }
        full_barrier();
        win_scan(st, w, tid, kNone, 0);
        continue;
      }
      if (tid == 0) { st.rsz[r2] = z2; st.rsum[r2] = w2; }
    }
    if (ne + total > st.Ecap) { status = ST_NEED_EDGES; break; }
    if (pool_used + total > st.pool_cap) { status = ST_NEED_POOL; break; }
    if (tid == 0) {
      w.seq[slot] = 0;
      st.order[3 * k + 0] = r0; st.order[3 * k + 1] = r1; st.order[3 * k + 2] = r2;
      st.sal_out[k] = root.sal;
      st.er[e].seq = 0;
    }
    if (tid >= 64 && tid < 128) w.touched[par][tid & 63] = 0;
    const bool small = total <= kMarkMax;

    win_stage_lists(st, s, tid, e, off0, len0, off1, len1, small);
    full_barrier();
    WPH(1);
    if (wn_now + total > st.wcap) {
#ifdef GLIA_HMT_PROFILE
      wcompacts += 1;
#endif
      const uint32_t wn_live = win_compact(w, tid, st.wcap);
      if (wn_live + total > st.wcap) {
        win_flush(st, w, tid);
        if (total > st.wcap) {
          if (tid == 0) { w.cthr = (int)st.wB; w.tsal = __builtin_inf(); w.tseq = ~0ull; }
          full_barrier();
        }
      }
    }
    const bool moved = wn_now + total > st.wcap;
    const WinTau tau = {moved ? w.cthr : cthr, moved ? w.tsal : tsal, moved ? w.tseq : tseq, smin, scale};
    const uint32_t nwork = small ? s.nitems : total;
    WPH(2);

    bool bad = false;
    uint32_t pend_e = kNone, pend_old = kNone;
    for (uint32_t base = 0; base < nwork; base += kGreedyThreads) {
      const uint32_t i = base + tid;
      if (i >= nwork) break;
      FatEntry f0, f1;
      bool h0, h1;
      uint32_t rs;
      if (!(small ? win_match<true>(st, s, i, e, off0, len0, off1, &rs, &h0, &h1, &f0, &f1) : win_match<false>(st, s, i, e, off0, len0, off1, &rs, &h0, &h1, &f0, &f1))) continue;
      const uint32_t idx = atomicAdd(&s.newcount, 1u);
      const uint32_t newE = (uint32_t)ne + idx;
      atomicOr(&w.touched[par][(rs >> 5) & 63u], 1u << (rs & 31u));
      double first;
      int second;
      if (mean_link(h0, f0.mean, (int)f0.n, h1, f1.mean, (int)f1.n, &first, &second)) bad = true;
      const uint32_t offRs = f0.off, posRs = f0.pos, lenRs = f0.len;
      if (h0 && h1) st.fpool[offRs + f1.pos].eid = kNone;
      const unsigned long long seq = update_seq(k, rs, r0, h0);
      const double sal = -first;
      store_new_edge(st, newE, rs, r2, posRs, idx, first, second, sal, seq, offRs, lenRs, r2off, 0u);
      if (small) { s.items[i] = offRs + posRs; s.newidx[i] = idx; }
      win_queue_edge<false>(st, w, tau, newE, sal, seq, rs, r2, make_uint2(offRs, lenRs), make_uint2(r2off, 0u), pend_e, pend_old);
      if (h0) win_retire_edge<false, COND, kKillMax>(st, tau, f0.eid, -f0.mean, &w.nk, w.kill, &w.kovf);
      if (h1) win_retire_edge<false, COND, kKillMax>(st, tau, f1.eid, -f1.mean, &w.nk, w.kill, &w.kovf);
    }
    if (bad) s.bad = 1;
    if (small) lds_barrier(); else full_barrier();
    if (s.bad) { if (pend_e != kNone) st.er[pend_e].next = pend_old; status = ST_BAD_SALIENCY; break; }
    WPH(3);
    const uint32_t newcount = s.newcount;
    if (small) {
      for (uint32_t i = tid; i < nwork; i += kGreedyThreads) { st.fpool[s.items[i]].len = newcount; st.er[(uint32_t)ne + s.newidx[i]].hv.y = newcount; }
    } else {
      win_complete_r2(st, tid, (uint32_t)ne, r2off, newcount);
    }
    if (w.kovf) full_barrier(); else lds_barrier();
    if (tid == 0) { st.adj_off[r2] = r2off; st.adj_len[r2] = newcount; s.nitems = 0; s.newcount = 0; }
    win_scan(st, w, tid, r2, newcount);
    if (pend_e != kNone) st.er[pend_e].next = pend_old;
    r2prev = r2;
    WPH(4);
#ifdef GLIA_HMT_PROFILE
    if (tid == 0) {
      const unsigned long long tn = __builtin_readcyclecounter();
      const int b = total <= 64 ? 0 : total <= 512 ? 1 : total <= kMarkMax ? 2 : total <= 8192 ? 3 : 4;
      wtb[b] += tn - wtiter; wnb[b] += 1; wdb[b] += total; wtiter = tn; winwin += w.n;
    }
#endif
    k += 1; ne += newcount; pool_used += total;
  }
#ifdef GLIA_HMT_PROFILE
  if (tid == 0) printf("[window profile] merges %llu: pop %llu  lists+table %llu  room %llu  build %llu  finish+scan %llu  loop-top %llu  reload %llu (cycles); reloads %llu (items %llu) compactions %llu dependent %llu; mean window fill %llu\n",
                       k, wph[0], wph[1], wph[2], wph[3], wph[4], wph[5], wph[6], wreloads, wloaded, wcompacts, wdeps, k ? winwin / k : 0ull);
  if (tid == 0) printf("[window profile] by width (<=64, <=512, <=1408, <=8192, more): merges %llu %llu %llu %llu %llu  cycles %llu %llu %llu %llu %llu  entries %llu %llu %llu %llu %llu\n",
                       wnb[0], wnb[1], wnb[2], wnb[3], wnb[4], wtb[0], wtb[1], wtb[2], wtb[3], wtb[4], wdb[0], wdb[1], wdb[2], wdb[3], wdb[4]);
#endif
  full_barrier();
  win_leave(st, w, tid, k, ne, pool_used, status);
}

}
}
```

Measured before the change: 310,200.

## Defer edge record writes below the window horizon and rebuild them from adjacency lists

After: 323,200, median of 6. 1.04x the previous value.

```diff
diff --git a/cli/edge_rebuild_check.cpp b/cli/edge_rebuild_check.cpp
--- /dev/null
+++ b/cli/edge_rebuild_check.cpp
@@ -0,0 +1,54 @@
+#include <cstdio>
+#include <cstring>
+#include <vector>
+#include "../glia_amd/csrc/edge_record.hpp"
+
+using namespace glia;
+
+int main() {
+  const uint32_t R = 5, R0 = 1;
+  struct E { uint32_t u, v, n; double mean; uint32_t r0; bool h0; };
+  const std::vector<E> edges = {{0, 1, 7, 0.125, 1, true},  {0, 2, 3, 0.5, 0, true},       {1, 2, 11, 0.33203125, 0, false}, {1, 3, 1, 0.0, 2, true},
+                                {2, 3, 40, 0.99609375, 1, false}, {0, 4, 5, 0.25, 3, true}, {2, 4, 9, 0.7421875, 2, true},    {3, 4, 2, 0.00390625, 1, true}};
+  std::vector<uint32_t> deg(R, 0), off(R, 0), cur(R, 0);
+  for (const E& e : edges) { ++deg[e.u]; ++deg[e.v]; }
+  for (uint32_t r = 1; r < R; ++r) off[r] = off[r - 1] + deg[r - 1];
+  std::vector<FatEntry> pool(2 * edges.size());
+  std::vector<uint32_t> posu(edges.size()), posv(edges.size());
+  for (size_t e = 0; e < edges.size(); ++e) {
+    const E& g = edges[e];
+    const uint32_t pu = cur[g.u]++, pv = cur[g.v]++;
+    FatEntry a; a.eid = (uint32_t)e; a.rs = g.v; a.n = g.n; a.pos = pv; a.off = off[g.v]; a.len = deg[g.v]; a.mean = g.mean;
+    FatEntry b = a; b.rs = g.u; b.pos = pu; b.off = off[g.u]; b.len = deg[g.u];
+    pool[off[g.u] + pu] = a; pool[off[g.v] + pv] = b;
+    posu[e] = pu; posv[e] = pv;
+  }
+  int checked = 0, cats[3] = {0, 0, 0};
+  for (uint32_t v = 0; v < R; ++v) {
+    for (uint32_t i = 0; i < deg[v]; ++i) {
+      const FatEntry& fe = pool[off[v] + i];
+      if (fe.eid == kRecNone || !(fe.rs < v)) continue;
+      const E& g = edges[fe.eid];
+      const uint32_t rs = g.u, r2 = g.v, k = r2 - R0;
+      const uint32_t cat = rs < g.r0 ? 0u : (g.h0 ? 1u : 2u);
+      const unsigned long long seq = ((unsigned long long)(k + 1u) << 32) | ((unsigned long long)cat << 30) | rs;
+      const double first = g.mean, sal = -first;
+      unsigned long long mb, sb;
+      memcpy(&mb, &first, 8); memcpy(&sb, &sal, 8);
+      const uint32_t want[16] = {rs, r2, posu[fe.eid], posv[fe.eid], (uint32_t)mb, (uint32_t)(mb >> 32), g.n, kRecNone,
+                                 off[rs], deg[rs], off[r2], deg[r2], (uint32_t)sb, (uint32_t)(sb >> 32), (uint32_t)seq, (uint32_t)(seq >> 32)};
+      const EdgeRec got = rebuild_edge_record(fe, i, v, off[v], deg[v], (uint32_t)((seq >> 30) & 3u), R0);
+      if (memcmp(&got, want, 64) != 0) {
+        const uint32_t* w = reinterpret_cast<const uint32_t*>(&got);
+        printf("edge_rebuild_check: edge %u (%u, %u) differs:", fe.eid, rs, r2);
+        for (int j = 0; j < 16; ++j) printf(" %08x/%08x", w[j], want[j]);
+        printf("\n");
+        return 1;
+      }
+      ++checked; ++cats[cat];
+    }
+  }
+  if (checked != (int)edges.size() || !cats[0] || !cats[1] || !cats[2]) { printf("edge_rebuild_check: %d of %zu edges visited\n", checked, edges.size()); return 1; }
+  printf("edge_rebuild_check: %d records rebuilt from list entries agree with the stored form (cat 0/1/2: %d/%d/%d)\n", checked, cats[0], cats[1], cats[2]);
+  return 0;
+}
diff --git a/glia_amd/csrc/edge_record.hpp b/glia_amd/csrc/edge_record.hpp
--- /dev/null
+++ b/glia_amd/csrc/edge_record.hpp
@@ -0,0 +1,48 @@
+#pragma once
+#include <stdint.h>
+
+#if defined(__HIPCC__)
+#define GLIA_REC_HD __host__ __device__
+#else
+#define GLIA_REC_HD
+#endif
+
+namespace glia {
+
+#if defined(__HIPCC__)
+typedef uint2 RecPair;
+#else
+struct RecPair { uint32_t x, y; };
+#endif
+constexpr uint32_t kRecNone = 0xFFFFFFFFu;
+
+struct __attribute__((aligned(16))) FatEntry {
+  uint32_t eid;
+  uint32_t rs;
+  uint32_t n;
+  uint32_t pos;
+  uint32_t off;
+  uint32_t len;
+  double mean;
+};
+static_assert(sizeof(FatEntry) == 32, "FatEntry layout");
+
+struct __attribute__((aligned(16))) EdgeRec {
+  uint32_t u, v, posu, posv;
+  double mean; int n; uint32_t next;
+  RecPair hu, hv;
+  double sal; unsigned long long seq;
+};
+static_assert(sizeof(EdgeRec) == 64, "EdgeRec layout");
+
+GLIA_REC_HD inline EdgeRec rebuild_edge_record(const FatEntry& fe, uint32_t idx, uint32_t v, uint32_t voff, uint32_t vlen, uint32_t cat, uint32_t R0) {
+  EdgeRec r;
+  r.u = fe.rs; r.v = v; r.posu = fe.pos; r.posv = idx;
+  r.mean = fe.mean; r.n = (int)fe.n; r.next = kRecNone;
+  r.hu.x = fe.off; r.hu.y = fe.len; r.hv.x = voff; r.hv.y = vlen;
+  r.sal = -fe.mean;
+  r.seq = ((unsigned long long)(v - R0 + 1u) << 32) | ((unsigned long long)(cat & 3u) << 30) | fe.rs;
+  return r;
+}
+
+}
diff --git a/glia_amd/csrc/greedy.hip b/glia_amd/csrc/greedy.hip
--- a/glia_amd/csrc/greedy.hip
+++ b/glia_amd/csrc/greedy.hip
@@ -70,6 +70,38 @@
   const uint32_t i = atomicAdd(counter, 1u);
   kseq[i] = q; vals[i] = e;
 }
+__global__ void win_collect_lists_kernel(WinState st, uint32_t n_regions, unsigned long long* kseq, uint32_t* vals, uint32_t cap, uint32_t* counter) {
+  const uint32_t r = (blockIdx.x * blockDim.x + threadIdx.x) >> 6, lane = threadIdx.x & 63u;
+  if (r >= n_regions || st.rdead[r]) return;
+  const uint32_t off = st.adj_off[r], len = st.adj_len[r];
+  const double smin = st.wrange[0], scale = st.wrange[1];
+  uint32_t rebuilt = 0;
+  for (uint32_t base = 0; base < len; base += 64u) {
+    const uint32_t i = base + lane;
+    unsigned long long q = 0;
+    uint32_t e = kNone;
+    if (i < len) {
+      const FatEntry fe = st.fpool[off + i];
+      if (fe.eid != kNone && fe.rs < r && !st.rdead[fe.rs]) {
+        e = fe.eid;
+        if ((unsigned long long)e >= st.ne_base && win_cell(-fe.mean, smin, scale, st.wB) < st.wch) {
+          const EdgeRec rec = rebuild_edge_record(fe, i, r, off, len, st.ecat[e], st.R0);
+          st.er[e] = rec;
+          q = rec.seq; ++rebuilt;
+        } else q = st.er[e].seq;
+      }
+    }
+    const unsigned long long m = __ballot(q != 0);
+    if (m == 0) continue;
+    const int first = (int)__builtin_ctzll(m);
+    uint32_t b0 = 0;
+    if ((int)lane == first) b0 = atomicAdd(&counter[0], (uint32_t)__popcll(m));
+    b0 = (uint32_t)__shfl((int)b0, first);
+    const uint32_t o = b0 + (uint32_t)__popcll(m & ((1ull << lane) - 1ull));
+    if (q != 0 && o < cap) { kseq[o] = q; vals[o] = e; }
+  }
+  if (rebuilt) atomicAdd(&counter[1], rebuilt);
+}
 __global__ void win_salkey_kernel(const EdgeRec* er, const uint32_t* vals, uint32_t n, unsigned long long* ksal) {
   const uint32_t i = blockIdx.x * blockDim.x + threadIdx.x;
   if (i < n) ksal[i] = f64_ord(er[vals[i]].sal);
@@ -115,6 +147,15 @@
   const EdgeRec r = er[e];
   g.e_u[e] = r.u; g.e_v[e] = r.v; g.e_posu[e] = r.posu; g.e_posv[e] = r.posv; g.e_mean[e] = r.mean; g.e_n[e] = r.n;
   g.pq.leaf_sal[e] = r.sal; g.pq.leaf_seq[e] = (rdead[r.u] | rdead[r.v]) ? 0ull : r.seq;
+}
+
+__global__ void edge_unpack_live(GreedyState g, const EdgeRec* er, const uint32_t* vals, uint32_t n) {
+  const uint32_t i = blockIdx.x * blockDim.x + threadIdx.x;
+  if (i >= n) return;
+  const uint32_t e = vals[i];
+  const EdgeRec r = er[e];
+  g.e_u[e] = r.u; g.e_v[e] = r.v; g.e_posu[e] = r.posu; g.e_posv[e] = r.posv; g.e_mean[e] = r.mean; g.e_n[e] = r.n;
+  g.pq.leaf_sal[e] = r.sal; g.pq.leaf_seq[e] = r.seq;
 }
 
 __global__ void edge_flags(const uint32_t* pa, const uint32_t* pb, long long P, uint32_t* flag, long long* partner) {
@@ -234,6 +275,8 @@
   long long prev_top_cell = -1;
   unsigned long long prev_ne = 0;
   double horizon_factor = 0.0;
+  bool from_lists = false;
+  unsigned long long rebuilt_last = 0;
 
   int init(DeviceBuffers& buf, WinState& ws, const double* leaf_sal, uint32_t n_initial, uint32_t B, uint32_t R, hipStream_t stream) {
     int rc;
@@ -253,7 +296,7 @@
     if ((rc = buf.get(&ksal2, E0, false, stream))) return rc;
     if ((rc = buf.get(&vals, E0, false, stream))) return rc;
     if ((rc = buf.get(&vals2, E0, false, stream))) return rc;
-    if ((rc = buf.get(&counter, 1, true, stream))) return rc;
+    if ((rc = buf.get(&counter, 2, true, stream))) return rc;
     GLIA_HIP_TRY(rocprim::radix_sort_pairs_desc(nullptr, tmp_bytes, kseq, kseq2, vals, vals2, (size_t)E0, 0, 64, stream));
     if ((rc = buf.get((char**)&tmp, tmp_bytes ? tmp_bytes : 16, false, stream))) return rc;
     ws.wrange = range; ws.isort = isort; ws.isort_seq = iseq; ws.ige = ige;
@@ -266,13 +309,21 @@
     GLIA_HIP_TRY(hipStreamSynchronize(stream));
     return GLIA_HMT_OK;
   }
+  int collect(const WinState& ws, uint32_t n_edges, uint32_t n_regions, hipStream_t stream, uint32_t* n_out) {
+    GLIA_HIP_TRY(hipMemsetAsync(counter, 0, 2 * sizeof(uint32_t), stream));
+    if (from_lists) hipLaunchKernelGGL(win_collect_lists_kernel, dim3((unsigned)(((unsigned long long)n_regions * 64ull + 255ull) / 256ull)), dim3(256), 0, stream, ws, n_regions, kseq, vals, E0, counter);
+    else hipLaunchKernelGGL(win_collect_kernel, dim3((n_edges + 255) / 256), dim3(256), 0, stream, ws.er, n_edges, ws.rdead, kseq, vals, counter);
+    GLIA_HIP_TRY(hipGetLastError());
+    uint32_t h[2] = {0, 0};
+    GLIA_HIP_TRY(hipMemcpyAsync(h, counter, sizeof(h), hipMemcpyDeviceToHost, stream));
+    GLIA_HIP_TRY(hipStreamSynchronize(stream));
+    if (h[0] > E0) { set_error("greedy: more live edges than initial edges (internal error)"); return GLIA_HMT_ERR_INTERNAL; }
+    *n_out = h[0]; rebuilt_last = h[1];
+    return GLIA_HMT_OK;
+  }
   int rebaseline(WinState& ws, uint32_t n_edges, unsigned long long* ctrl, hipStream_t stream) {
-    GLIA_HIP_TRY(hipMemsetAsync(counter, 0, sizeof(uint32_t), stream));
-    hipLaunchKernelGGL(win_collect_kernel, dim3((n_edges + 255) / 256), dim3(256), 0, stream, ws.er, n_edges, ws.rdead, kseq, vals, counter);
     uint32_t n = 0;
-    GLIA_HIP_TRY(hipMemcpyAsync(&n, counter, sizeof(uint32_t), hipMemcpyDeviceToHost, stream));
-    GLIA_HIP_TRY(hipStreamSynchronize(stream));
-    if (n > E0) { set_error("greedy: more live edges than initial edges (internal error)"); return GLIA_HMT_ERR_INTERNAL; }
+    if (int rc = collect(ws, n_edges, ws.R0 + (uint32_t)ctrl[CTRL_MERGES], stream, &n)) return rc;
     if (n) {
       size_t bytes = tmp_bytes;
       GLIA_HIP_TRY(rocprim::radix_sort_pairs_desc(tmp, bytes, kseq, kseq2, vals, vals2, (size_t)n, 0, 64, stream));
@@ -346,6 +397,7 @@
   if (window) {
     if ((rc = entries.add(buf, &ws.fpool, st.pool_cap, stream))) return rc;
     if ((rc = edges.add(buf, &ws.er, st.Ecap, stream))) return rc;
+    if ((rc = edges.add(buf, &ws.ecat, st.Ecap, stream))) return rc;
   }
   else if ((rc = entries.add(buf, &st.pool, st.pool_cap, stream))) return rc;
   if ((rc = edges.add(buf, &st.e_u, st.Ecap, stream)) || (rc = edges.add(buf, &st.e_v, st.Ecap, stream)) ||
@@ -425,6 +477,7 @@
     ws.cond_n = st.cond_n; ws.cond_t0 = st.cond_t0; ws.cond_t1 = st.cond_t1; ws.cond_rpb = st.cond_rpb;
     if ((rc = base.init(buf, ws, st.pq.leaf_sal, E0, B, R, stream))) return rc;
     if (req.cond_n <= 0 && !batch_off) base.horizon_factor = option("GLIA_HMT_HORIZON", &o_txt) ? atof(o_txt.c_str()) : 0.5;
+    base.from_lists = req.cond_n <= 0 && !batch_off;
     if ((rc = base.rebaseline(ws, E0, ctrl, stream))) return rc;
   } else if ((rc = pq_setup(buf, st.pq, stream))) return rc;
   GLIA_HIP_TRY(hipMemcpyAsync(st.ctrl, ctrl, sizeof(ctrl), hipMemcpyHostToDevice, stream));
@@ -450,7 +503,8 @@
     GLIA_HIP_TRY(hipGetLastError());
     GLIA_HIP_TRY(hipMemcpyAsync(ctrl, st.ctrl, sizeof(ctrl), hipMemcpyDeviceToHost, stream));
     GLIA_HIP_TRY(hipStreamSynchronize(stream));
-    if (trace) fprintf(stderr, "[trace] merge loop launch ended: status %llu, merges %llu of %u regions, edges %llu, list entries %llu\n", ctrl[CTRL_STATUS], ctrl[CTRL_MERGES], R, ctrl[CTRL_EDGES], ctrl[CTRL_ENTRIES]);
+    if (trace) fprintf(stderr, "[trace] merge loop launch ended: status %llu, merges %llu of %u regions, edges %llu, list entries %llu, records rebuilt %llu\n", ctrl[CTRL_STATUS], ctrl[CTRL_MERGES], R, ctrl[CTRL_EDGES], ctrl[CTRL_ENTRIES], base.rebuilt_last);
+    base.rebuilt_last = 0;
     if (ctrl[CTRL_STATUS] == ST_DONE) break;
     switch (ctrl[CTRL_STATUS]) {
       case ST_RUN:
@@ -471,8 +525,15 @@
         if (!window) return unhandled();
         entries.remove(&ws.fpool);
         edges.remove(&ws.er);
+        edges.remove(&ws.ecat);
         if ((rc = entries.add(buf, &st.pool, st.pool_cap, stream))) return rc;
         hipLaunchKernelGGL(fat_to_thin, dim3((unsigned)((ctrl[CTRL_ENTRIES] + 255) / 256)), dim3(256), 0, stream, ws.fpool, st.pool, ctrl[CTRL_ENTRIES]);
+        if (base.from_lists) {
+          uint32_t n_live = 0;
+          if ((rc = base.collect(ws, (uint32_t)ctrl[CTRL_EDGES], R + (uint32_t)ctrl[CTRL_MERGES], stream, &n_live))) return rc;
+          hipLaunchKernelGGL(fill_leaves_dead, dim3((st.Ecap + 255) / 256), dim3(256), 0, stream, st.pq, 0u);
+          if (n_live) hipLaunchKernelGGL(edge_unpack_live, dim3((n_live + 255) / 256), dim3(256), 0, stream, st, ws.er, base.vals, n_live);
+        } else
         hipLaunchKernelGGL(edge_unpack, dim3((unsigned)((ctrl[CTRL_EDGES] + 255) / 256)), dim3(256), 0, stream, st, ws.er, ws.rdead, (uint32_t)ctrl[CTRL_EDGES]);
         GLIA_HIP_TRY(hipGetLastError());
         if ((rc = pq_setup(buf, st.pq, stream))) return rc;
diff --git a/glia_amd/csrc/greedy_batch.hpp b/glia_amd/csrc/greedy_batch.hpp
--- a/glia_amd/csrc/greedy_batch.hpp
+++ b/glia_amd/csrc/greedy_batch.hpp
@@ -149,6 +149,7 @@
 
 #ifdef GLIA_HMT_PROFILE
 __device__ unsigned long long g_wideprof[8];
+__device__ unsigned long long g_edgeprof[3][2];
 #define WIDE_T(i) do { if (tid == 0) { const unsigned long long tn_ = __builtin_readcyclecounter(); g_wideprof[i] += tn_ - wt_; wt_ = tn_; } } while (0)
 #else
 #define WIDE_T(i) do {} while (0)
@@ -185,6 +186,9 @@
   const uint32_t lenR2 = small ? nwork : 0u;
   bool bad = false;
   uint32_t pend_e = kNone, pend_old = kNone;
+#ifdef GLIA_HMT_PROFILE
+  uint32_t ep_above = 0, ep_below = 0;
+#endif
   auto rounds = [&](auto small_tag) {
     constexpr bool SMALL = decltype(small_tag)::value;
     for (uint32_t base = 0; base < nwork; base += kGreedyThreads) {
@@ -203,8 +207,12 @@
       if (h0 && h1) st.fpool[offRs + f1.pos].eid = kNone;
       const unsigned long long seq = update_seq(k, rs, r0, h0);
       const double sal = -first;
-      store_new_edge(st, newE, rs, r2, posRs, idx, first, second, sal, seq, offRs, lenRs, r2off, lenR2);
-      win_queue_edge<true>(st, w, tau, newE, sal, seq, rs, r2, make_uint2(offRs, lenRs), make_uint2(r2off, lenR2), pend_e, pend_old);
+      const uint32_t cell = win_cell(sal, tau.smin, tau.scale, st.wB);
+#ifdef GLIA_HMT_PROFILE
+      if (cell < st.wch) ++ep_below; else ++ep_above;
+#endif
+      store_new_edge<true>(st, newE, rs, r2, posRs, idx, first, second, sal, seq, offRs, lenRs, r2off, lenR2, cell);
+      win_queue_edge<true>(st, w, tau, newE, sal, seq, rs, r2, make_uint2(offRs, lenRs), make_uint2(r2off, lenR2), cell, pend_e, pend_old);
       if (h0) win_retire_edge<true, false, kBatchKill>(st, tau, f0.eid, -f0.mean, &b.nkill, b.kill, &b.kovf);
       if (h1) win_retire_edge<true, false, kBatchKill>(st, tau, f1.eid, -f1.mean, &b.nkill, b.kill, &b.kovf);
     }
@@ -215,12 +223,16 @@
   if (small) lds_barrier(); else full_barrier();
   WIDE_T(4);
   const uint32_t newcount = s.newcount;
-  if (!small) win_complete_r2(st, tid, (uint32_t)ne, r2off, newcount);
+  if (!small) win_complete_r2<true>(st, tid, (uint32_t)ne, r2off, newcount, smin, scale);
   if (!small) for (uint32_t i = tid; i < (w.n < st.wcap ? w.n : st.wcap); i += kGreedyThreads) if (w.v[i] == r2) w.hv[i].y = newcount;
   if (pend_e != kNone) st.er[pend_e].next = pend_old;
   if (tid == 0) { st.adj_off[r2] = r2off; st.adj_len[r2] = newcount; }
   lds_barrier();
   WIDE_T(5);
+#ifdef GLIA_HMT_PROFILE
+  if (ep_above) atomicAdd(&g_edgeprof[small ? 1 : 2][0], (unsigned long long)ep_above);
+  if (ep_below) atomicAdd(&g_edgeprof[small ? 1 : 2][1], (unsigned long long)ep_below);
+#endif
   if (tid == 0) { s.nitems = 0; s.newcount = 0; }
   *newcount_out = newcount;
   return total;
@@ -250,6 +262,7 @@
 #ifdef GLIA_HMT_PROFILE
   unsigned long long bph[8] = {0, 0, 0, 0, 0, 0, 0, 0}, blast = __builtin_readcyclecounter(), brounds = 0, bmembers = 0, bvalid = 0, bwide = 0, bcut_sal = 0, bcut_dep = 0;
   unsigned long long bw_n[4] = {0, 0, 0, 0}, bw_cyc[4] = {0, 0, 0, 0}, bw_ent[4] = {0, 0, 0, 0}, bw_new[4] = {0, 0, 0, 0};
+  uint32_t bep_above = 0, bep_below = 0;
   unsigned long long bsel[2] = {0, 0}, bsel_n[2] = {0, 0};
 #define BPH0(wide) do { if (tid == 0) { unsigned long long tn = __builtin_readcyclecounter(); bph[0] += tn - blast; bsel[wide] += tn - blast; bsel_n[wide] += 1; blast = tn; } } while (0)
 #define BPH(i) do { if (tid == 0) { unsigned long long tn = __builtin_readcyclecounter(); bph[i] += tn - blast; blast = tn; } } while (0)
@@ -442,8 +455,12 @@
         if (both[p]) st.fpool[offRs + p_pos[p]].eid = kNone;
         const unsigned long long seq = update_seq(kk, rs, r0, h0);
         const double sal = -first[p];
-        store_new_edge(st, newE, rs, r2, posRs, idx[p], first[p], second[p], sal, seq, offRs, lenRs, r2off, newcount);
-        win_queue_edge<true>(st, w, tau, newE, sal, seq, rs, r2, make_uint2(offRs, lenRs), make_uint2(r2off, newcount), pend_e, pend_old);
+        const uint32_t cell = win_cell(sal, tau.smin, tau.scale, st.wB);
+#ifdef GLIA_HMT_PROFILE
+        if (cell < st.wch) ++bep_below; else ++bep_above;
+#endif
+        store_new_edge<true>(st, newE, rs, r2, posRs, idx[p], first[p], second[p], sal, seq, offRs, lenRs, r2off, newcount, cell);
+        win_queue_edge<true>(st, w, tau, newE, sal, seq, rs, r2, make_uint2(offRs, lenRs), make_uint2(r2off, newcount), cell, pend_e, pend_old);
         win_retire_edge<true, false, kBatchKill>(st, tau, fe[p].eid, -fe[p].mean, &b.nkill, b.kill, &b.kovf);
         if (both[p]) win_retire_edge<true, false, kBatchKill>(st, tau, p_eid[p], -p_mean[p], &b.nkill, b.kill, &b.kovf);
       }
@@ -459,6 +476,12 @@
     BPH(4);
   }
 #ifdef GLIA_HMT_PROFILE
+  if (bep_above) atomicAdd(&g_edgeprof[0][0], (unsigned long long)bep_above);
+  if (bep_below) atomicAdd(&g_edgeprof[0][1], (unsigned long long)bep_below);
+  full_barrier();
+  if (tid == 0) printf("[batch profile] created edges at or above / below the horizon (cumulative): narrow commit %llu / %llu  wide on the LDS table %llu / %llu  wide on the global marks %llu / %llu\n",
+                       atomicAdd(&g_edgeprof[0][0], 0ull), atomicAdd(&g_edgeprof[0][1], 0ull), atomicAdd(&g_edgeprof[1][0], 0ull), atomicAdd(&g_edgeprof[1][1], 0ull),
+                       atomicAdd(&g_edgeprof[2][0], 0ull), atomicAdd(&g_edgeprof[2][1], 0ull));
   if (tid == 0) printf("[batch profile] merges %llu: select %llu  compute %llu  validate %llu  commit %llu  scan %llu  loop-top %llu  reload %llu (cycles); rounds %llu candidates %llu committed %llu (cut by saliency %llu, by adjacency %llu) wide %llu\n",
                        k, bph[0], bph[1], bph[2], bph[3], bph[4], bph[5], bph[6], brounds, bmembers, bvalid, bcut_sal, bcut_dep, bwide);
   if (tid == 0) printf("[batch profile] scan phases (cumulative cycles, wave 0): loads %llu  compare %llu  top2 %llu  top2 with a tied best %llu  barrier %llu  calls %llu  tied second %llu  tied best %llu\n",
diff --git a/glia_amd/csrc/greedy_window.hpp b/glia_amd/csrc/greedy_window.hpp
--- a/glia_amd/csrc/greedy_window.hpp
+++ b/glia_amd/csrc/greedy_window.hpp
@@ -1,27 +1,11 @@
 #pragma once
 #include "greedy_tree.hpp"
+#include "edge_record.hpp"
 
 namespace glia {
-
-struct __attribute__((aligned(16))) FatEntry {
-  uint32_t eid;
-  uint32_t rs;
-  uint32_t n;
-  uint32_t pos;
-  uint32_t off;
-  uint32_t len;
-  double mean;
-};
-
 namespace {
 
-struct __attribute__((aligned(16))) EdgeRec {
-  uint32_t u, v, posu, posv;
-  double mean; int n; uint32_t next;
-  uint2 hu, hv;
-  double sal; unsigned long long seq;
-};
-static_assert(sizeof(EdgeRec) == 64, "EdgeRec layout");
+static_assert(kRecNone == kNone, "edge_record.hpp");
 struct WinState {
   EdgeRec* er; FatEntry* fpool;
   uint32_t* whead;
@@ -40,6 +24,7 @@
   uint32_t wch;
   uint8_t* rdead;
   unsigned long long force_tree;
+  uint8_t* ecat;
 };
 constexpr uint32_t kWinCap = 1536;
 constexpr uint32_t kWinBudget = 768;
@@ -385,15 +370,19 @@
   }
   return true;
 }
+template <bool BATCH>
 __device__ __forceinline__ void store_new_edge(const WinState& st, uint32_t newE, uint32_t rs, uint32_t r2, uint32_t posRs, uint32_t idx, double first, int second,
-                                               double sal, unsigned long long seq, uint32_t offRs, uint32_t lenRs, uint32_t r2off, uint32_t lenR2) {
-  uint4* pq4 = reinterpret_cast<uint4*>(&st.er[newE]);
-  pq4[0] = make_uint4(rs, r2, posRs, idx);
-  const unsigned long long mb = (unsigned long long)__double_as_longlong(first);
-  pq4[1] = make_uint4((uint32_t)mb, (uint32_t)(mb >> 32), (uint32_t)second, kNone);
-  pq4[2] = make_uint4(offRs, lenRs, r2off, lenR2);
-  const unsigned long long sbits = (unsigned long long)__double_as_longlong(sal);
-  pq4[3] = make_uint4((uint32_t)sbits, (uint32_t)(sbits >> 32), (uint32_t)seq, (uint32_t)(seq >> 32));
+                                               double sal, unsigned long long seq, uint32_t offRs, uint32_t lenRs, uint32_t r2off, uint32_t lenR2, uint32_t cell) {
+  if (BATCH && cell < st.wch) st.ecat[newE] = (uint8_t)((uint32_t)(seq >> 30) & 3u);
+  else {
+    uint4* pq4 = reinterpret_cast<uint4*>(&st.er[newE]);
+    pq4[0] = make_uint4(rs, r2, posRs, idx);
+    const unsigned long long mb = (unsigned long long)__double_as_longlong(first);
+    pq4[1] = make_uint4((uint32_t)mb, (uint32_t)(mb >> 32), (uint32_t)second, kNone);
+    pq4[2] = make_uint4(offRs, lenRs, r2off, lenR2);
+    const unsigned long long sbits = (unsigned long long)__double_as_longlong(sal);
+    pq4[3] = make_uint4((uint32_t)sbits, (uint32_t)(sbits >> 32), (uint32_t)seq, (uint32_t)(seq >> 32));
+  }
   FatEntry a; a.eid = newE; a.rs = r2; a.n = (uint32_t)second; a.pos = idx; a.off = r2off; a.len = lenR2; a.mean = first;
   st.fpool[offRs + posRs] = a;
   FatEntry b; b.eid = newE; b.rs = rs; b.n = (uint32_t)second; b.pos = posRs; b.off = offRs; b.len = lenRs; b.mean = first;
@@ -401,8 +390,7 @@
 }
 template <bool BATCH>
 __device__ __forceinline__ void win_queue_edge(const WinState& st, WinShared& w, const WinTau& tau, uint32_t newE, double sal, unsigned long long seq, uint32_t rs, uint32_t r2,
-                                               uint2 hrs, uint2 hr2, uint32_t& pend_e, uint32_t& pend_old) {
-  const uint32_t cell = win_cell(sal, tau.smin, tau.scale, st.wB);
+                                               uint2 hrs, uint2 hr2, uint32_t cell, uint32_t& pend_e, uint32_t& pend_old) {
   const bool above = win_above(tau.cthr, tau.tsal, tau.tseq, (int)cell, sal, seq);
   uint32_t sl = kWinCap;
   if (above) {
@@ -429,11 +417,12 @@
     const uint32_t j = atomicAdd(nkill, 1u); if (j < KMAX) kill[j] = de; else *kovf = 1;
   } else atomicSub(&st.wcnt[dc], 1u);
 }
-__device__ __forceinline__ void win_complete_r2(const WinState& st, int tid, uint32_t ne, uint32_t r2off, uint32_t newcount) {
+template <bool BATCH>
+__device__ __forceinline__ void win_complete_r2(const WinState& st, int tid, uint32_t ne, uint32_t r2off, uint32_t newcount, double smin, double scale) {
   for (uint32_t j = tid; j < newcount; j += kGreedyThreads) {
     const FatEntry fb = st.fpool[r2off + j];
     st.fpool[fb.off + fb.pos].len = newcount;
-    st.er[ne + j].hv.y = newcount;
+    if (!BATCH || win_cell(-fb.mean, smin, scale, st.wB) >= st.wch) st.er[ne + j].hv.y = newcount;
     st.mark0[fb.rs] = 0; st.mark1[fb.rs] = 0;
   }
 }
@@ -581,9 +570,10 @@
       if (h0 && h1) st.fpool[offRs + f1.pos].eid = kNone;
       const unsigned long long seq = update_seq(k, rs, r0, h0);
       const double sal = -first;
-      store_new_edge(st, newE, rs, r2, posRs, idx, first, second, sal, seq, offRs, lenRs, r2off, 0u);
+      const uint32_t cell = win_cell(sal, tau.smin, tau.scale, st.wB);
+      store_new_edge<false>(st, newE, rs, r2, posRs, idx, first, second, sal, seq, offRs, lenRs, r2off, 0u, cell);
       if (small) { s.items[i] = offRs + posRs; s.newidx[i] = idx; }
-      win_queue_edge<false>(st, w, tau, newE, sal, seq, rs, r2, make_uint2(offRs, lenRs), make_uint2(r2off, 0u), pend_e, pend_old);
+      win_queue_edge<false>(st, w, tau, newE, sal, seq, rs, r2, make_uint2(offRs, lenRs), make_uint2(r2off, 0u), cell, pend_e, pend_old);
       if (h0) win_retire_edge<false, COND, kKillMax>(st, tau, f0.eid, -f0.mean, &w.nk, w.kill, &w.kovf);
       if (h1) win_retire_edge<false, COND, kKillMax>(st, tau, f1.eid, -f1.mean, &w.nk, w.kill, &w.kovf);
     }
@@ -595,7 +585,7 @@
     if (small) {
       for (uint32_t i = tid; i < nwork; i += kGreedyThreads) { st.fpool[s.items[i]].len = newcount; st.er[(uint32_t)ne + s.newidx[i]].hv.y = newcount; }
     } else {
-      win_complete_r2(st, tid, (uint32_t)ne, r2off, newcount);
+      win_complete_r2<false>(st, tid, (uint32_t)ne, r2off, newcount, smin, scale);
     }
     if (w.kovf) full_barrier(); else lds_barrier();
     if (tid == 0) { st.adj_off[r2] = r2off; st.adj_len[r2] = newcount; s.nitems = 0; s.newcount = 0; }
```
